# SunBangjie/FYP-BidirectionalPathTracer

Measured on AMD Instinct MI355X. Metric: Mrays/s + RMSE vs the scalar oracle, BDPT pass, Sponza-class scene 1920x1080 depth 8, higher is better.
Workload: dtype f32

## Files before the change

### fyp-bidirectionalpathtracer_amd/csrc/api.cpp

```cpp
#include <hip/hip_runtime.h>

#include <cmath>
#include <cstdio>
#include <cstdlib>
#include <cstring>
#include <future>
#include <functional>
#include <atomic>
#include <chrono>
#include <string>
#include <thread>
#include <vector>

#include "../../include/bdpt.h"
#include <new>

#include "bvh.h"
#include "kernels.h"
#include "refit.h"
#include "skin.h"
#include "scene_bvh.h"

using namespace bdpt;

namespace {
constexpr int kMaxStages = 64;
constexpr size_t kCountBlocks = 1;
constexpr size_t kHeadBlocks = 2;
constexpr size_t kLazyBlocks = kMaxLazyRounds + 2;
constexpr size_t kEyeCountBlock = kLazyBlocks - 1;
static_assert(kEyeCountBlock > (size_t)kMaxLazyRounds, "the eye list's cursor block must be one no lazy round uses");
constexpr size_t kCursorWords = (kCountBlocks + kHeadBlocks + kLazyBlocks) * kCursorBlock + 4 * kRayCursorBlock;
}

struct bdpt_ctx {
  int device = 0;
  int numCUs = 256;
  std::string err;
  bool haveScene = false, haveCamera = false, haveSize = false;
  SceneDev S{};
  std::vector<void*> sceneAllocs;
  bdpt_bvh_info bvhInfo{};
  bdpt_camera cam{};
  bdpt_environment env{};
  uint32_t W = 0, H = 0, maxDepth = 0;
  std::vector<std::pair<uint32_t, uint32_t>> rowRanges;
  uint32_t tileRows = 0;
  SplatLayout sl{1, 1, 0};
  bdpt_stripes stripes{0, 1, 0};
  PathBuf P{};
  std::vector<void*> frameAllocs;
  unsigned long long* splat = nullptr;
  unsigned long long* ownSplat = nullptr;
  DevCounters* counters = nullptr;
  hipStream_t lastStream = nullptr;
  bool timing = false;
  hipEvent_t ev[kMaxStages + 1]{};
  const char* stageNames[kMaxStages]{};
  int numStages = 0;
  bool evCreated = false;
  static constexpr int kMaxSideStages = 4;
  hipEvent_t sideEv[2 * kMaxSideStages]{};
  const char* sideNames[kMaxSideStages]{};
  int numSideStages = 0;
  int lazyRounds = 3;
  LaunchGrids grids{};
  int* stackOvf = nullptr;
  uint32_t stackOvfStride = 0;
  unsigned long long* rayCursor = nullptr;
  unsigned long long* adaptiveSum = nullptr;
  bdpt_gbuffer ownGb{};
  float4* bmfrPos[2] = {nullptr, nullptr};
  float4* bmfrNorm[2] = {nullptr, nullptr};
  float4* bmfrNoisy[2] = {nullptr, nullptr};
  float4* bmfrFiltered[2] = {nullptr, nullptr};
  uint8_t* bmfrAccept = nullptr;
  uint32_t* bmfrPrevPixel = nullptr;
  int bmfrRead = 0;
  hipStream_t walkStream = nullptr;
  hipEvent_t evFork = nullptr, evJoin = nullptr, evSplat = nullptr;
  uint32_t* hintPix = nullptr;
  bool hints = true;
  bdpt_camera hintCam{};
  bool hintCamValid = false;
  uint32_t numVertices = 0, numTriangles = 0;
  uint32_t* lightMaps = nullptr;
  bool refitReady = false;
  BvhRefitPlan refitPlan;
  RefitDev refit{};
  uint32_t numUpdates = 0;
  float* stage[3] = {nullptr, nullptr, nullptr};
  void* pinned = nullptr;
  size_t pinnedBytes = 0;
  hipEvent_t evStage = nullptr, evOrder = nullptr;
  bool stageInFlight = false;
  unsigned long long* groupSplat = nullptr;
  uint32_t groupSplatPlanes = 0;
  uint8_t* groupLightIdx = nullptr;
  const uint32_t* alphaTris = nullptr;
  uint32_t numAlphaTris = 0;
  bool areaReady = false;
  AreaDev area{};
  uint32_t areaTextured = 0;
  float* areaBlockSum = nullptr;
  uint32_t* areaBlockLast = nullptr;
  std::vector<void*> skinAllocs;
  bool haveSkin = false;
  SkinDev skin{};
  float* skinPalette[2] = {nullptr, nullptr};
};

namespace {

template <class F>
void hostParallelFor(size_t n, const F& f) {
  const int threads = bvhBuildThreads();
  if (threads <= 1 || n < 65536) {
    f((size_t)0, n);
    return;
  }
  WorkerScope pool;
  const size_t chunk = (n + (size_t)threads - 1) / (size_t)threads;
  for (int t = 1; t < threads; t++) {
    const size_t a = std::min(n, chunk * (size_t)t), b = std::min(n, a + chunk);
    if (a < b) pool.spawn([&f, a, b] { f(a, b); });
  }
  f((size_t)0, std::min(n, chunk));
  pool.join();
}

std::vector<uint32_t> alphaQuadPlane(const bdpt_texture& t) {
  std::vector<uint32_t> q((size_t)t.width * t.height);
  hostParallelFor(t.height, [&](size_t y0, size_t y1) { alphaQuadRows(t.rgba8, t.width, t.height, (uint32_t)y0, (uint32_t)y1, q.data()); });
  return q;
}

bool fail(bdpt_ctx* c, const std::string& m) {
  if (c) c->err = m;
  return false;
}
#define HIPCHK(ctx, expr)                                                                       \
  do {                                                                                          \
    hipError_t e_ = (expr);                                                                     \
    if (e_ != hipSuccess) {                                                                     \
      fail(ctx, std::string(#expr) + ": " + hipGetErrorString(e_));                             \
      return BDPT_E_HIP;                                                                        \
    }                                                                                           \
  } while (0)

template <class T>
int devAlloc(bdpt_ctx* c, std::vector<void*>& pool, T** out, size_t count) {
  void* p = nullptr;
  size_t bytes = std::max<size_t>(count * sizeof(T), 16);
  hipError_t e = hipMalloc(&p, bytes);
  if (e != hipSuccess) {
    fail(c, std::string("hipMalloc(") + std::to_string(bytes) + "): " + hipGetErrorString(e));
    return BDPT_E_NOMEM;
  }
  pool.push_back(p);
  *out = reinterpret_cast<T*>(p);
  return BDPT_OK;
}
template <class T>
int devUpload(bdpt_ctx* c, std::vector<void*>& pool, const T** out, const T* host, size_t count) {
  T* d = nullptr;
  int rc = devAlloc(c, pool, &d, count);
  if (rc) return rc;
  if (count) {
    std::string e;
    if (!bvhUploadStaged(d, host, count * sizeof(T), e)) {
      fail(c, e);
      return BDPT_E_HIP;
    }
  }
  *out = d;
  return BDPT_OK;
}
void freePool(std::vector<void*>& pool) {
  for (void* p : pool) (void)hipFree(p);
  pool.clear();
}
void freeLightGroups(bdpt_ctx* c) {
  if (c->groupSplat) (void)hipFree(c->groupSplat);
  if (c->groupLightIdx) (void)hipFree(c->groupLightIdx);
  c->groupSplat = nullptr;
  c->groupSplatPlanes = 0;
  c->groupLightIdx = nullptr;
}

#define ENTER(ctx) HIPCHK(ctx, hipSetDevice((ctx)->device))

bool streamIsCapturing(hipStream_t st) {
  hipStreamCaptureStatus cs = hipStreamCaptureStatusNone;
  if (hipStreamIsCapturing(st, &cs) != hipSuccess) return false;
  return cs != hipStreamCaptureStatusNone;
}

int allocOwnGbuffer(bdpt_ctx* c) {
  if (c->ownGb.worldPosition) return BDPT_OK;
  const size_t n = (size_t)c->W * c->H;
  const size_t mark = c->frameAllocs.size();
  bdpt_gbuffer g{};
  int rc;
  if ((rc = devAlloc(c, c->frameAllocs, &g.worldPosition, n * 4)) || (rc = devAlloc(c, c->frameAllocs, &g.worldNormal, n * 4)) ||
      (rc = devAlloc(c, c->frameAllocs, &g.materialDiffuse, n * 4)) || (rc = devAlloc(c, c->frameAllocs, &g.materialSpecRough, n * 4)) ||
      (rc = devAlloc(c, c->frameAllocs, &g.materialExtraParams, n * 4)) || (rc = devAlloc(c, c->frameAllocs, &g.emissive, n * 4))) {
    while (c->frameAllocs.size() > mark) {
      (void)hipFree(c->frameAllocs.back());
      c->frameAllocs.pop_back();
    }
    return rc;
  }
  c->ownGb = g;
  return BDPT_OK;
}

int allocBmfrHistory(bdpt_ctx* c) {
  if (c->bmfrAccept) return BDPT_OK;
  const size_t n = (size_t)c->W * c->H;
  const size_t mark = c->frameAllocs.size();
  float4 *pos[2]{}, *norm[2]{}, *noisy[2]{}, *filt[2]{};
  uint8_t* accept = nullptr;
  uint32_t* prevPixel = nullptr;
  int rc = BDPT_OK;
  for (int k = 0; k < 2 && !rc; k++) {
    if ((rc = devAlloc(c, c->frameAllocs, &pos[k], n)) || (rc = devAlloc(c, c->frameAllocs, &norm[k], n)) ||
        (rc = devAlloc(c, c->frameAllocs, &noisy[k], n)) || (rc = devAlloc(c, c->frameAllocs, &filt[k], n)))
      break;
  }
  if (!rc) rc = devAlloc(c, c->frameAllocs, &accept, n);
  if (!rc) rc = devAlloc(c, c->frameAllocs, &prevPixel, n);
  if (rc) {
    while (c->frameAllocs.size() > mark) {
      (void)hipFree(c->frameAllocs.back());
      c->frameAllocs.pop_back();
    }
    return rc;
  }
  for (int k = 0; k < 2; k++) {
    c->bmfrPos[k] = pos[k];
    c->bmfrNorm[k] = norm[k];
    c->bmfrNoisy[k] = noisy[k];
    c->bmfrFiltered[k] = filt[k];
  }
  c->bmfrAccept = accept;
  c->bmfrPrevPixel = prevPixel;
  return bdpt_bmfr_reset(c);
}

void stageMark(bdpt_ctx* c, hipStream_t st, const char* name) {
  if (!c->timing || c->numStages >= kMaxStages) return;
  c->stageNames[c->numStages] = name;
  c->numStages++;
  (void)hipEventRecord(c->ev[c->numStages], st);
}
void sideBegin(bdpt_ctx* c, hipStream_t side, const char* name) {
  if (!c->timing || c->numSideStages >= bdpt_ctx::kMaxSideStages) return;
  c->sideNames[c->numSideStages] = name;
  (void)hipEventRecord(c->sideEv[2 * c->numSideStages], side);
}
void sideEnd(bdpt_ctx* c, hipStream_t side) {
  if (!c->timing || c->numSideStages >= bdpt_ctx::kMaxSideStages) return;
  (void)hipEventRecord(c->sideEv[2 * c->numSideStages + 1], side);
  c->numSideStages++;
}

}

extern "C" {

int bdpt_create(int device_ordinal, bdpt_ctx** out_ctx) {
  if (!out_ctx) return BDPT_E_INVALID;
  *out_ctx = nullptr;
  int n = 0;
  if (hipGetDeviceCount(&n) != hipSuccess || n <= 0 || device_ordinal < 0 || device_ordinal >= n) return BDPT_E_HIP;
  if (hipSetDevice(device_ordinal) != hipSuccess) return BDPT_E_HIP;
  bdpt_ctx* c = new bdpt_ctx();
  c->device = device_ordinal;
  hipDeviceProp_t prop;
  if (hipGetDeviceProperties(&prop, device_ordinal) == hipSuccess && prop.multiProcessorCount > 0)
    c->numCUs = prop.multiProcessorCount;
  if (hipStreamCreateWithFlags(&c->walkStream, hipStreamNonBlocking) != hipSuccess ||
      hipEventCreateWithFlags(&c->evFork, hipEventDisableTiming) != hipSuccess ||
      hipEventCreateWithFlags(&c->evJoin, hipEventDisableTiming) != hipSuccess ||
      hipEventCreateWithFlags(&c->evSplat, hipEventDisableTiming) != hipSuccess ||
      hipEventCreateWithFlags(&c->evStage, hipEventDisableTiming) != hipSuccess ||
      hipEventCreateWithFlags(&c->evOrder, hipEventDisableTiming) != hipSuccess) {
    bdpt_destroy(c);
    return BDPT_E_HIP;
  }
  c->stackOvfStride = (uint32_t)c->numCUs * kMaxPersistentPerCU * kWave;
  if (kStackOvfRows > 0 &&
      hipMalloc(reinterpret_cast<void**>(&c->stackOvf), (size_t)kStackOvfRows * c->stackOvfStride * sizeof(int)) != hipSuccess) {
    bdpt_destroy(c);
    return BDPT_E_NOMEM;
  }
  if (hipMalloc(reinterpret_cast<void**>(&c->rayCursor), 2 * sizeof(unsigned long long)) != hipSuccess ||
      hipMemset(c->rayCursor, 0, 2 * sizeof(unsigned long long)) != hipSuccess ||
      hipMalloc(reinterpret_cast<void**>(&c->adaptiveSum), 2 * sizeof(unsigned long long)) != hipSuccess ||
      hipMemset(c->adaptiveSum, 0, 2 * sizeof(unsigned long long)) != hipSuccess) {
    bdpt_destroy(c);
    return BDPT_E_NOMEM;
  }
  bvhPrewarmStaging(device_ordinal);
  *out_ctx = c;
  return BDPT_OK;
}

void bdpt_destroy(bdpt_ctx* c) {
  if (!c) return;
  (void)hipSetDevice(c->device);
  (void)hipDeviceSynchronize();
  if (c->stackOvf) (void)hipFree(c->stackOvf);
  if (c->rayCursor) (void)hipFree(c->rayCursor);
  if (c->adaptiveSum) (void)hipFree(c->adaptiveSum);
  freeLightGroups(c);
  freePool(c->sceneAllocs);
  freePool(c->skinAllocs);
  freePool(c->frameAllocs);
  if (c->evCreated)
    for (int i = 0; i <= kMaxStages; i++) (void)hipEventDestroy(c->ev[i]);
  if (c->evCreated)
    for (hipEvent_t e : c->sideEv) (void)hipEventDestroy(e);
  if (c->evFork) (void)hipEventDestroy(c->evFork);
  if (c->evJoin) (void)hipEventDestroy(c->evJoin);
  if (c->evSplat) (void)hipEventDestroy(c->evSplat);
  if (c->evStage) (void)hipEventDestroy(c->evStage);
  if (c->evOrder) (void)hipEventDestroy(c->evOrder);
  if (c->pinned) (void)hipHostFree(c->pinned);
  if (c->walkStream) (void)hipStreamDestroy(c->walkStream);
  delete c;
}

const char* bdpt_last_error(const bdpt_ctx* c) { return c ? c->err.c_str() : "null context"; }

// ... 895 lines not shown
  c->lastStream = st;
  return BDPT_OK;
}

static_assert(sizeof(bdpt_light_sample) == 48 && sizeof(bdpt_light_emit) == 48 && offsetof(bdpt_light_sample, status) == 46,
              "the light query kernels write a record as three float4, light and status sharing the last word");
int bdpt_light_query(bdpt_ctx* c, const bdpt_light_desc* d, void* stream) {
  if (!c || !d) return BDPT_E_INVALID;
  if (!c->haveScene) {
    fail(c, "light_query: no scene (bdpt_set_scene first)");
    return BDPT_E_STATE;
  }
  const bool emitMode = d->mode == BDPT_LIGHT_EMIT;
  if (d->mode > BDPT_LIGHT_EMIT || d->matIndex > 1 || (d->flags & ~(BDPT_PARAM_AREA_LIGHTS | BDPT_LIGHT_USE_HINTS))) {
    fail(c, "light_query: unknown mode or flags, or matIndex > 1");
    return BDPT_E_INVALID;
  }
  const bool compact = d->compactRays || d->compactItems || d->compactCount;
  if (emitMode && (compact || (d->flags & BDPT_LIGHT_USE_HINTS))) {
    fail(c, "light_query: compaction and BDPT_LIGHT_USE_HINTS go with BDPT_LIGHT_NEE");
    return BDPT_E_INVALID;
  }
  if (compact && !(d->compactRays && d->compactItems && d->compactCount)) {
    fail(c, "light_query: compactRays, compactItems and compactCount go together");
    return BDPT_E_INVALID;
  }
  if (!d->num) return BDPT_OK;
  if (!aligned(d->seeds, 4) || (d->seedsOut && !aligned(d->seedsOut, 4)) || (d->numDevice && !aligned(d->numDevice, 4)) ||
      (emitMode ? !aligned(d->emits, 16) : (!aligned(d->surfaces, 16) || !aligned(d->samples, 16))) ||
      (compact && (!aligned(d->compactRays, 16) || !aligned(d->compactItems, 4) || !aligned(d->compactCount, 4)))) {
    fail(c, "light_query: surfaces, seeds, samples, emits or a compaction buffer missing or not aligned (records 16 bytes, words 4)");
    return BDPT_E_INVALID;
  }
  ENTER(c);
  hipStream_t st = reinterpret_cast<hipStream_t>(stream);
  AreaDev A{};
  if (d->flags & BDPT_PARAM_AREA_LIGHTS) {
    if (int rc = ensureAreaLights(c, st)) return rc;
    A = c->area;
  }
  if (int rc = orderAfterLast(c, st)) return rc;
  LightQueryDev Q{};
  Q.surf = reinterpret_cast<const float4*>(d->surfaces);
  Q.seeds = d->seeds;
  Q.seedsOut = d->seedsOut;
  Q.out = emitMode ? reinterpret_cast<float4*>(d->emits) : reinterpret_cast<float4*>(d->samples);
  Q.cap = d->num;
  Q.count = d->numDevice;
  Q.minT = d->minT;
  Q.compactRays = reinterpret_cast<float4*>(d->compactRays);
  Q.compactItems = d->compactItems;
  Q.compactCount = d->compactCount;
  launchLightQuery(c->S, Q, A, emitMode, d->matIndex == 0, (d->flags & BDPT_LIGHT_USE_HINTS) != 0, st);
  HIPCHK(c, hipGetLastError());
  c->lastStream = st;
  return BDPT_OK;
}

static_assert(sizeof(bdpt_connect_sample) == 48 && sizeof(bdpt_camera_sample) == 64 && offsetof(bdpt_connect_sample, status) == 44 &&
                  offsetof(bdpt_camera_sample, G) == 44 && offsetof(bdpt_camera_sample, pixel) == 48,
              "the connection query kernels write a record as three / four float4");
int bdpt_connect_query(bdpt_ctx* c, const bdpt_connect_desc* d, void* stream) {
  if (!c || !d) return BDPT_E_INVALID;
  if (!c->haveScene) {
    fail(c, "connect_query: no scene (bdpt_set_scene first)");
    return BDPT_E_STATE;
  }
  if (d->mode > BDPT_CONNECT_CAMERA || d->matIndex > 1 || d->flags || d->reserved) {
    fail(c, "connect_query: unknown mode, non-zero flags or reserved, or matIndex > 1");
    return BDPT_E_INVALID;
  }
  const bool camMode = d->mode == BDPT_CONNECT_CAMERA;
  if (camMode && !c->haveCamera) {
    fail(c, "connect_query: BDPT_CONNECT_CAMERA without a camera (bdpt_set_camera first)");
    return BDPT_E_STATE;
  }
  if (camMode && (!d->width || !d->height || (uint64_t)d->width * d->height >= (1ull << 32))) {
    fail(c, "connect_query: width and height must be > 0 with width * height < 2^32");
    return BDPT_E_INVALID;
  }
  const bool compact = d->compactRays || d->compactItems || d->compactCount;
  if (compact && !(d->compactRays && d->compactItems && d->compactCount)) {
    fail(c, "connect_query: compactRays, compactItems and compactCount go together");
    return BDPT_E_INVALID;
  }
  if (!d->num) return BDPT_OK;
  if (!aligned(d->light, 16) || (d->numDevice && !aligned(d->numDevice, 4)) ||
      (camMode ? !aligned(d->cameraSamples, 16)
               : (!aligned(d->eye, 16) || !aligned(d->samples, 16) || (d->eyePrev && !aligned(d->eyePrev, 16)) ||
                  (d->lightPrev && !aligned(d->lightPrev, 16)))) ||
      (compact && (!aligned(d->compactRays, 16) || !aligned(d->compactItems, 4) || !aligned(d->compactCount, 4)))) {
    fail(c, "connect_query: eye, light, samples, a predecessor or a compaction buffer missing or not aligned (records 16 bytes, words 4)");
    return BDPT_E_INVALID;
  }
  ENTER(c);
  hipStream_t st = reinterpret_cast<hipStream_t>(stream);
  if (int rc = orderAfterLast(c, st)) return rc;
  ConnectQueryDev Q{};
  Q.light = reinterpret_cast<const float4*>(d->light);
  Q.lightSpecular = d->lightSpecular;
  if (camMode) {
    Q.out = reinterpret_cast<float4*>(d->cameraSamples);
    Q.width = d->width;
    Q.height = d->height;
    Q.jitter[0] = d->pixelJitter[0];
    Q.jitter[1] = d->pixelJitter[1];
  } else {
    Q.eye = reinterpret_cast<const float4*>(d->eye);
    Q.eyePrev = reinterpret_cast<const float4*>(d->eyePrev);
    Q.lightPrev = reinterpret_cast<const float4*>(d->lightPrev);
    Q.eyeSpecular = d->eyeSpecular;
    Q.out = reinterpret_cast<float4*>(d->samples);
  }
  Q.cap = d->num;
  Q.count = d->numDevice;
  Q.minT = d->minT;
  Q.compactRays = reinterpret_cast<float4*>(d->compactRays);
  Q.compactItems = d->compactItems;
  Q.compactCount = d->compactCount;
  launchConnectQuery(Q, camMode ? &c->cam : nullptr, d->matIndex == 0, st);
  HIPCHK(c, hipGetLastError());
  c->lastStream = st;
  return BDPT_OK;
}

int bdpt_splat_add(bdpt_ctx* c, const bdpt_splat_desc* d, void* stream) {
  if (!c || !d) return BDPT_E_INVALID;
  if (!d->num) return BDPT_OK;
  if (!aligned(d->pixels, 4) || !aligned(d->values, 16) || !aligned(d->splat, 16) || (d->items && !aligned(d->items, 4)) ||
      (d->numDevice && !aligned(d->numDevice, 4))) {
    fail(c, "splat_add: pixels, values, splat, items or numDevice missing or not aligned (splat and values 16 bytes, words 4)");
    return BDPT_E_INVALID;
  }
  ENTER(c);
  hipStream_t st = reinterpret_cast<hipStream_t>(stream);
  if (int rc = orderAfterLast(c, st)) return rc;
  SplatAddDev A{};
  A.pixels = d->pixels;
  A.values = reinterpret_cast<const float4*>(d->values);
  A.visible = d->visible;
  A.items = d->items;
  A.splat = reinterpret_cast<unsigned long long*>(d->splat);
  A.numPixels = d->numPixels;
  A.cap = d->num;
  A.count = d->numDevice;
  launchSplatAdd(A, st);
  HIPCHK(c, hipGetLastError());
  c->lastStream = st;
  return BDPT_OK;
}

int bdpt_get_refit_info(bdpt_ctx* c, bdpt_refit_info* out) {
  if (!c || !out) return BDPT_E_INVALID;
  if (!c->haveScene) return BDPT_E_STATE;
  ENTER(c);
  *out = bdpt_refit_info{};
  out->sahCostBuilt = c->bvhInfo.sahCost;
  out->sahCost = c->bvhInfo.sahCost;
  out->numUpdates = c->numUpdates;
  if (c->numUpdates == 0) return BDPT_OK;
  HIPCHK(c, hipDeviceSynchronize());
  std::vector<float> area((size_t)c->refit.numNodes * 4);
  float root[6] = {0, 0, 0, 0, 0, 0};
  if (c->refit.numNodes) {
    HIPCHK(c, hipMemcpy(area.data(), c->refit.childArea, area.size() * sizeof(float), hipMemcpyDeviceToHost));
    HIPCHK(c, hipMemcpy(root, c->refit.box, sizeof(root), hipMemcpyDeviceToHost));
  }
  out->sahCost = bvhRefitSah(c->refitPlan, root, area.data());
  return BDPT_OK;
}

int bdpt_ctx_recs_hash(bdpt_ctx* c, uint64_t* out_hash) {
  if (!c || !out_hash) return BDPT_E_INVALID;
  if (!c->haveScene) return BDPT_E_STATE;
  ENTER(c);
  HIPCHK(c, hipDeviceSynchronize());
  std::vector<BvhRec> recs(c->S.numRecs);
  HIPCHK(c, hipMemcpy(recs.data(), c->S.recs, recs.size() * sizeof(BvhRec), hipMemcpyDeviceToHost));
  uint64_t h = 1469598103934665603ull;
  const uint8_t* b = reinterpret_cast<const uint8_t*>(recs.data());
  for (size_t i = 0; i < recs.size() * sizeof(BvhRec); i++) h = (h ^ b[i]) * 1099511628211ull;
  *out_hash = h;
  return BDPT_OK;
}

namespace {
int resizeRows(bdpt_ctx* c, uint32_t width, uint32_t height, uint32_t maxDepth);
}

int bdpt_resize(bdpt_ctx* c, uint32_t width, uint32_t height, bdpt_tile tile, uint32_t maxDepth) {
  if (!c) return BDPT_E_INVALID;
  if (!width || !height || tile.y0 > tile.y1 || tile.y1 > height) {
    fail(c, "resize: bad frame or tile");
    return BDPT_E_INVALID;
  }
  c->rowRanges.clear();
  if (tile.y1 > tile.y0) c->rowRanges.push_back({tile.y0, tile.y1});
  c->tileRows = tile.y1 - tile.y0;
  c->stripes = bdpt_stripes{0, 1, 0};
  c->sl = SplatLayout{1, 1, height};
  return resizeRows(c, width, height, maxDepth);
}

int bdpt_resize_stripes(bdpt_ctx* c, uint32_t width, uint32_t height, bdpt_stripes st, uint32_t maxDepth) {
  if (!c) return BDPT_E_INVALID;
  if (!width || !height || !st.stripeRows || !st.numOwners || st.owner >= st.numOwners) {
    fail(c, "resize_stripes: bad frame or stripe description");
    return BDPT_E_INVALID;
  }
  c->rowRanges.clear();
  c->tileRows = 0;
  const uint32_t numStripes = (height + st.stripeRows - 1) / st.stripeRows;
  for (uint32_t s = st.owner; s < numStripes; s += st.numOwners) {
    const uint32_t a = s * st.stripeRows, b = std::min(height, a + st.stripeRows);
    c->rowRanges.push_back({a, b});
    c->tileRows += b - a;
  }
  c->stripes = st;
  c->sl = SplatLayout{st.stripeRows, st.numOwners, ((numStripes + st.numOwners - 1) / st.numOwners) * st.stripeRows};
  return resizeRows(c, width, height, maxDepth);
}

uint32_t bdpt_stripe_rows(uint32_t height, uint32_t numOwners) {
  const uint32_t per = height / std::max(1u, numOwners * 4u);
  return std::max(1u, std::min(8u, per));
}
int bdpt_get_tile_info(const bdpt_ctx* c, bdpt_tile_info* out) {
  if (!c || !out) return BDPT_E_INVALID;
  if (!c->haveSize) return BDPT_E_STATE;
  out->numRows = c->tileRows;
  out->numPixels = c->P.Np;
  out->chunkRows = c->sl.chunkRows;
  out->numRowRanges = (uint32_t)c->rowRanges.size();
  out->splatU64 = (uint64_t)c->sl.owners * c->sl.chunkRows * c->W * 4;
  out->chunkU64 = (uint64_t)c->sl.chunkRows * c->W * 4;
  return BDPT_OK;
}

int bdpt_tile_row_ranges(const bdpt_ctx* c, uint32_t* out_first_last, uint32_t cap) {
  if (!c || !out_first_last) return BDPT_E_INVALID;
  if (!c->haveSize) return BDPT_E_STATE;
  const uint32_t n = std::min<uint32_t>(cap, (uint32_t)c->rowRanges.size());
  for (uint32_t i = 0; i < n; i++) {
    out_first_last[2 * i] = c->rowRanges[i].first;
    out_first_last[2 * i + 1] = c->rowRanges[i].second;
  }
  return (int)n;
}

namespace {
int resizeRows(bdpt_ctx* c, uint32_t width, uint32_t height, uint32_t maxDepth) {
  if (maxDepth > BDPT_MAX_DEPTH) {
    fail(c, "resize: maxDepth exceeds BDPT_MAX_DEPTH");
    return BDPT_E_LIMIT;
  }
  if ((uint64_t)width * height >= (1ull << 32) || (uint64_t)c->sl.owners * c->sl.chunkRows * width >= (1ull << 32)) {
    fail(c, "resize: frame too large");
    return BDPT_E_LIMIT;
  }
  if ((uint64_t)c->tileRows * width >= (1ull << 24)) {
    fail(c, "resize: a tile holds at most 2^24 - 1 pixels (path ids pack the pixel in 24 bits); render in smaller tiles");
    return BDPT_E_LIMIT;
  }
  HIPCHK(c, hipSetDevice(c->device));
  HIPCHK(c, hipDeviceSynchronize());
  freePool(c->frameAllocs);
  freeLightGroups(c);
  for (int k = 0; k < 2; k++) c->bmfrPos[k] = c->bmfrNorm[k] = c->bmfrNoisy[k] = c->bmfrFiltered[k] = nullptr;
  c->ownGb = bdpt_gbuffer{};
  c->bmfrAccept = nullptr;
  c->bmfrPrevPixel = nullptr;
  c->haveSize = false;
  c->W = width;
  c->H = height;
  c->maxDepth = maxDepth;
  PathBuf P{};
  P.Np = c->tileRows * width;
  P.D1 = std::max<uint32_t>(maxDepth, 1) + 1;
  const size_t np = std::max<uint32_t>(P.Np, 1);
  int rc;
  {
    std::vector<uint32_t> pix;
    pix.reserve(np);
    for (const auto& rr : c->rowRanges)
      for (uint32_t y = rr.first; y < rr.second; y++)
        for (uint32_t x = 0; x < width; x++) pix.push_back(y * width + x);
    if ((rc = devUpload(c, c->frameAllocs, &P.pix, pix.data(), pix.size()))) return rc;
  }
  if ((rc = devAlloc(c, c->frameAllocs, &P.v, (size_t)2 * P.D1 * NF4 * 4 * np))) return rc;
  if ((rc = devAlloc(c, c->frameAllocs, &P.rayDir, (size_t)6 * np))) return rc;
  if ((rc = devAlloc(c, c->frameAllocs, &P.seedE, np))) return rc;
  if ((rc = devAlloc(c, c->frameAllocs, &P.seedL, np))) return rc;
  if ((rc = devAlloc(c, c->frameAllocs, &P.eyeLast, np))) return rc;
  if ((rc = devAlloc(c, c->frameAllocs, &P.lightLast, np))) return rc;
  if ((rc = devAlloc(c, c->frameAllocs, &P.lightReal, np))) return rc;
  P.pathSubCap = (uint32_t)((((np + kWave - 1) / kWave + kNumSubQueues - 1) / kNumSubQueues + 1) * kWave);
  const size_t qcap = (size_t)P.pathSubCap * kNumSubQueues;
  for (int q = 0; q < 3; q++)
    if ((rc = devAlloc(c, c->frameAllocs, &P.queue[q], qcap))) return rc;
  if ((rc = devAlloc(c, c->frameAllocs, &P.qcount, (size_t)kCursorWords))) return rc;
  P.qhead = P.qcount + kCountBlocks * kCursorBlock;
  P.lazyCount = P.qhead + kHeadBlocks * kCursorBlock;
  P.rayCount = P.lazyCount + kLazyBlocks * kCursorBlock;
  P.rayHead = P.rayCount + 2 * kRayCursorBlock;
  {
    const uint32_t D = std::max<uint32_t>(maxDepth, 1);
    const uint64_t slots = (uint64_t)2 * D + numConnectPairs(D);
    const uint64_t blocks = (np + kWave - 1) / kWave;
    const uint64_t queueGridBlocks = (uint64_t)(P.pathSubCap / kWave) * kNumSubQueues;
    const uint64_t pairs = std::max<uint32_t>(numConnectPairs(D), 1);
    uint64_t subCapTerms = 0, subCapPairs = ((queueGridBlocks + kNumRaySubQueues - 1) / kNumRaySubQueues) * kWave * pairs;
    {
      const uint64_t G = D > 8 ? 16 : 8;
      const uint64_t perSub = (queueGridBlocks * G + kNumRaySubQueues - 1) / kNumRaySubQueues;
      subCapTerms = std::max<uint64_t>(subCapTerms, perSub * kWave * 2);
      subCapPairs = std::max<uint64_t>(subCapPairs, perSub * (kWave / G) * pairs);
    }
    (void)blocks;
    const uint64_t cap = (subCapTerms + subCapPairs) * kNumRaySubQueues;
    if (cap >= (1ull << 32) - 1) {
      fail(c, "resize: shadow-ray queue would exceed 2^32 entries; render in smaller tiles");
      return BDPT_E_LIMIT;
    }
    P.raySubCap[RAY_TERMS] = (uint32_t)subCapTerms;
    P.raySubCap[RAY_PAIRS] = (uint32_t)subCapPairs;
    P.rayBase[RAY_TERMS] = 0;
    P.rayBase[RAY_PAIRS] = (uint32_t)(subCapTerms * kNumRaySubQueues);
    P.rayCap = (uint32_t)cap;
    if ((rc = devAlloc(c, c->frameAllocs, &P.rayQ, (size_t)7 * cap))) return rc;
    if ((rc = devAlloc(c, c->frameAllocs, &P.rayContrib, (size_t)3 * cap))) return rc;
    if ((rc = devAlloc(c, c->frameAllocs, &P.rayVis, (size_t)cap))) return rc;
    if ((rc = devAlloc(c, c->frameAllocs, &P.slotRay, (size_t)slots * np))) return rc;
    if ((rc = devAlloc(c, c->frameAllocs, &P.splatPix, (size_t)D * np))) return rc;
    c->lazyRounds = np >= (1u << 18) ? 3 : 2;
    if (const char* e = std::getenv("BDPT_LAZY_ROUNDS")) {
      const int v = std::atoi(e);
      if (v >= 1 && v <= kMaxLazyRounds) c->lazyRounds = v;
    }
    const uint32_t batch = numConnectPairs(D);
    if ((rc = devAlloc(c, c->frameAllocs, &P.misE, (size_t)(D + 1) * np))) return rc;
    if ((rc = devAlloc(c, c->frameAllocs, &P.misL, (size_t)(D + 1) * np))) return rc;
    if ((rc = devAlloc(c, c->frameAllocs, &P.lazyCursor, np))) return rc;
    if ((rc = devAlloc(c, c->frameAllocs, &P.lazyRay, (size_t)std::max<uint32_t>(batch, 1) * np))) return rc;
  }
  c->hintPix = nullptr;
  c->hintCamValid = false;
  if (std::getenv("BDPT_NO_HINTS") == nullptr) {
    if ((rc = devAlloc(c, c->frameAllocs, &c->hintPix, (size_t)width * height))) return rc;
    HIPCHK(c, hipMemset(c->hintPix, 0xFF, (size_t)width * height * sizeof(uint32_t)));
  }
  const size_t splatU64 = (size_t)c->sl.owners * c->sl.chunkRows * width * 4;
  if ((rc = devAlloc(c, c->frameAllocs, &c->ownSplat, splatU64))) return rc;
  c->splat = c->ownSplat;
  if ((rc = devAlloc(c, c->frameAllocs, &c->counters, 1))) return rc;
  HIPCHK(c, hipMemset(c->splat, 0, splatU64 * sizeof(unsigned long long)));
  HIPCHK(c, hipMemset(c->counters, 0, sizeof(DevCounters)));
  c->P = P;
  if (!c->evCreated) {
    for (int i = 0; i <= kMaxStages; i++) HIPCHK(c, hipEventCreate(&c->ev[i]));
    for (hipEvent_t& e : c->sideEv) HIPCHK(c, hipEventCreate(&e));
    c->evCreated = true;
  }
  c->haveSize = true;
  return BDPT_OK;
}
}

int bdpt_gbuffer_execute(bdpt_ctx* c, const bdpt_gbuffer_params* gp, const bdpt_gbuffer* out, void* stream) {
  if (!c || !gp || !out) return BDPT_E_INVALID;
  if (!c->haveScene || !c->haveCamera || !c->haveSize) {
    fail(c, "gbuffer_execute: scene, camera and size must be set first");
    return BDPT_E_STATE;
  }
  if (!out->worldPosition || !out->worldNormal || !out->materialDiffuse || !out->materialSpecRough ||
      !out->materialExtraParams || !out->emissive) {
    fail(c, "gbuffer_execute: all six channels are required");
    return BDPT_E_INVALID;
  }
  ENTER(c);
  hipStream_t st = reinterpret_cast<hipStream_t>(stream);
  GBufferDev G{};
  G.cam = c->cam;
  G.gp = *gp;
  G.W = c->W;
  G.H = c->H;
  G.Np = c->P.Np;
  G.pix = c->P.pix;
  G.gb = *out;
  G.counters = nullptr;
  G.hintPix = c->hintPix;
  if (c->hintPix && c->tileRows != c->H && (!c->hintCamValid || std::memcmp(&c->hintCam, &c->cam, sizeof(bdpt_camera)) != 0)) {
    GBufferDev A = G;
    A.Np = c->W * c->H;
    A.pix = nullptr;
    launchHintFill(c->S, A, st);
    c->hintCam = c->cam;
    c->hintCamValid = true;
  }
  launchGBuffer(c->S, G, st);
  HIPCHK(c, hipGetLastError());
  c->lastStream = st;
  return BDPT_OK;
}

namespace {
int frameSetup(bdpt_ctx* c, const bdpt_params* p, const bdpt_gbuffer* in, float* out, hipStream_t st, FrameDev& F) {
  if (!c || !p || !out) return BDPT_E_INVALID;
  ENTER(c);
  if (!in) {
    if (!c->haveSize) {
      fail(c, "execute: scene, camera and size must be set first");
      return BDPT_E_STATE;
    }
    if (!c->ownGb.worldPosition) {
      if (streamIsCapturing(st)) {
        fail(c, "execute: the built-in primary stage needs bdpt_prepare(BDPT_PREPARE_PRIMARY) before stream capture");
        return BDPT_E_STATE;
      }
      if (int rc = allocOwnGbuffer(c)) return rc;
    }
    in = &c->ownGb;
  }
  if (!c->haveScene || !c->haveCamera || !c->haveSize) {
    fail(c, "execute: scene, camera and size must be set first");
    return BDPT_E_STATE;
  }
  if (p->maxDepth > c->maxDepth) {
    fail(c, "execute: params.maxDepth exceeds the depth given to bdpt_resize");
    return BDPT_E_LIMIT;
  }
  if (p->matIndex > 1) {
    fail(c, "execute: matIndex must be 0 (GGX) or 1 (Lambertian)");
    return BDPT_E_INVALID;
  }
  if (!in->worldPosition || !in->worldNormal || !in->materialDiffuse || !in->materialSpecRough || !in->emissive) {
    fail(c, "execute: G-buffer channels missing");
    return BDPT_E_INVALID;
  }
  F = FrameDev{};
  F.cam = c->cam;
  F.p = *p;
  F.W = c->W;
  F.H = c->H;
  F.sl = c->sl;
  F.out = out;
  F.splat = c->splat;
  F.gb = *in;
  F.counters = c->counters;
  F.envMap = c->env.envMap;
  F.envW = c->env.width;
  F.envH = c->env.height;
  for (int k = 0; k < 3; k++) F.envColor[k] = c->env.color[k];
  F.hintPix = c->hintPix;
  return BDPT_OK;
}

int connectionTail(bdpt_ctx* c, const FrameDev& F, hipStream_t st, const FrameVariant& V) {
  const PathBuf& P = c->P;
  const bdpt_params* p = &F.p;
  const int D = (int)p->maxDepth;
  if (!(p->flags & BDPT_PARAM_NO_CONNECT) && D >= 2) {
    const int nPairs = (int)numConnectPairs((uint32_t)D);
    const int b0 = (nPairs + kLazyBatchDiv - 1) / kLazyBatchDiv;
    int left = nPairs;
    for (int r = 0; r < c->lazyRounds && left > 0; r++) {
      const int batch = (r + 1 == c->lazyRounds) ? left : (b0 < left ? b0 : left);
      left -= batch;
      uint32_t* list = P.queue[1 + (r & 1)];
      uint32_t* next = P.queue[1 + ((r + 1) & 1)];
      HIPCHK(c, hipMemsetAsync(P.rayCount + (size_t)RAY_PAIRS * kRayCursorBlock, 0, kRayCursorBlock * sizeof(uint32_t), st));
      HIPCHK(c, hipMemsetAsync(P.rayHead + (size_t)RAY_PAIRS * kRayCursorBlock, 0, kRayCursorBlock * sizeof(uint32_t), st));
      launchLazyGen(F, P, list, P.lazyCount + (size_t)r * kCursorBlock, batch, st);
      stageMark(c, st, "lazy_gen");
      launchTraceShadow(c->S, F, P, RAY_PAIRS, c->grids, c->numCUs, st);
      stageMark(c, st, "lazy_trace");
      launchLazyCheck(F, P, V, list, P.lazyCount + (size_t)r * kCursorBlock, batch, next, P.lazyCount + (size_t)(r + 1) * kCursorBlock,
                      st);
    }
    stageMark(c, st, "lazy_check");
  }
  if (!(p->flags & BDPT_PARAM_DEFER_RESOLVE)) {
    launchFrameResolve(F, P, V, st);
    stageMark(c, st, V.kind == FrameKind::Groups ? "resolve_groups" : V.kind == FrameKind::Masked ? "resolve_masked" : "resolve");
  }
  HIPCHK(c, hipGetLastError());
  c->lastStream = st;
  return BDPT_OK;
}
}

namespace {
int executeFrame(bdpt_ctx* c, const bdpt_params* p, const bdpt_gbuffer* in, float* out, void* stream, const FrameVariant& V0,
                 bool groupsTakeArea = false) {
  FrameDev F;
  hipStream_t st = reinterpret_cast<hipStream_t>(stream);
  if (int rc = frameSetup(c, p, in, out, st, F)) return rc;
  FrameVariant V = V0;
  if (p->flags & BDPT_PARAM_AREA_LIGHTS) {
    if (p->flags & (BDPT_PARAM_MIS_POWER | BDPT_PARAM_MIS_LINEAR)) {
      fail(c, "execute: BDPT_PARAM_AREA_LIGHTS is not supported with BDPT_PARAM_MIS_POWER / _LINEAR");
      return BDPT_E_INVALID;
    }
    if (V.kind == FrameKind::Groups && !groupsTakeArea) {
      fail(c, "light groups: BDPT_PARAM_AREA_LIGHTS is not supported (the group planes have no slot for area lights)");
      return BDPT_E_INVALID;
    }
    if (int rc = ensureAreaLights(c, st)) return rc;
    V.area = c->area;
    if (V.kind == FrameKind::Groups && V.area.n) V.groups.areaW = V.area.total;
  }
  const PathBuf& P = c->P;
  PathBuf PE = P;
  if (V.kind == FrameKind::Masked) {
    PE.queue[0] = V.mask.eye;
    PE.qcount = V.mask.eyeCount;
  }
  if (!in) {
    bdpt_gbuffer_params gp{};
    gp.pixelJitter[0] = p->pixelJitter[0];
    gp.pixelJitter[1] = p->pixelJitter[1];
    gp.focalLen = 1.0f;
    gp.frameCount = p->frameCount;
    gp.envColor[0] = gp.envColor[1] = 0.5f;
    gp.envColor[2] = 0.8f;
    gp.envColor[3] = 1.0f;
    if (int rc = bdpt_gbuffer_execute(c, &gp, &c->ownGb, stream)) return rc;
  }

  c->numStages = 0;
  c->numSideStages = 0;
  if (c->timing) HIPCHK(c, hipEventRecord(c->ev[0], st));
  HIPCHK(c, hipMemsetAsync(P.qcount, 0, (size_t)kCursorWords * sizeof(uint32_t), st));
  HIPCHK(c, hipMemsetAsync(c->splat, 0, (size_t)c->sl.owners * c->sl.chunkRows * c->W * 4 * sizeof(unsigned long long), st));
  if (V.kind == FrameKind::Groups)
    HIPCHK(c, hipMemsetAsync(V.groups.splat, 0, (size_t)V.groups.numGroups * V.groups.framePix * 4 * sizeof(unsigned long long), st));
  if (!(p->flags & BDPT_PARAM_KEEP_COUNTERS)) HIPCHK(c, hipMemsetAsync(c->counters, 0, sizeof(DevCounters), st));
  stageMark(c, st, "clear");

  launchInitPaths(c->S, F, P, V, st);
  stageMark(c, st, "init_paths");

  launchWalk(c->S, F, P, V, c->grids, c->numCUs, st);
  stageMark(c, st, "walk");

  const bool mis = (p->flags & (BDPT_PARAM_MIS_POWER | BDPT_PARAM_MIS_LINEAR)) != 0;
  if (mis) {
    launchMisPrefix(F, P, st);
    stageMark(c, st, "mis_prefix");
    launchGenNee(c->S, F, PE, V.area, st);
    stageMark(c, st, "gen_nee");
    launchGenSplat(c->S, F, P, st);
    stageMark(c, st, "gen_splat");
    launchGenConnect(c->S, F, PE, st);
    stageMark(c, st, "gen_connect");
    launchTraceShadow(c->S, F, P, RAY_TERMS, c->grids, c->numCUs, st);
    stageMark(c, st, "trace_terms");
  } else {
    HIPCHK(c, hipEventRecord(c->evFork, st));
    HIPCHK(c, hipStreamWaitEvent(c->walkStream, c->evFork, 0));
    sideBegin(c, c->walkStream, "side:gen_splat");
    launchGenSplat(c->S, F, P, c->walkStream);
    sideEnd(c, c->walkStream);
    HIPCHK(c, hipEventRecord(c->evSplat, c->walkStream));
    sideBegin(c, c->walkStream, "side:gen_connect");
    launchGenConnect(c->S, F, PE, c->walkStream);
    sideEnd(c, c->walkStream);
    HIPCHK(c, hipEventRecord(c->evJoin, c->walkStream));
    launchGenNee(c->S, F, PE, V.area, st);
    stageMark(c, st, "gen_nee");
    HIPCHK(c, hipStreamWaitEvent(st, c->evSplat, 0));
    stageMark(c, st, "splat_wait");
    launchTraceShadow(c->S, F, P, RAY_TERMS, c->grids, c->numCUs, st);
    stageMark(c, st, "trace_terms");
    HIPCHK(c, hipStreamWaitEvent(st, c->evJoin, 0));
    stageMark(c, st, "connect_wait");
  }
  launchTraceShadow(c->S, F, P, RAY_PAIRS, c->grids, c->numCUs, st);
  stageMark(c, st, "trace_pairs");
  launchGather(F, P, V, P.queue[1], P.lazyCount, st);
  stageMark(c, st, "gather");
  if (p->flags & BDPT_PARAM_DEFER_TAIL) {
    HIPCHK(c, hipGetLastError());
    c->lastStream = st;
    return BDPT_OK;
  }
  return connectionTail(c, F, st, V);
}

int allocLightGroups(bdpt_ctx* c, hipStream_t st, uint32_t planes) {
  if (c->groupSplat && c->groupSplatPlanes >= planes) return BDPT_OK;
  if (streamIsCapturing(st)) {
    fail(c, "light groups: the splat planes need bdpt_prepare(BDPT_PREPARE_LIGHT_GROUPS / _LIGHT_GROUP_TABLE) before stream capture");
    return BDPT_E_STATE;
  }
  if (c->groupSplat) {
    HIPCHK(c, hipDeviceSynchronize());
    freeLightGroups(c);
  }
  const size_t n = (size_t)c->W * c->H;
  void *sp = nullptr, *li = nullptr;
  if (hipMalloc(&sp, std::max<size_t>((size_t)planes * n * 4 * sizeof(unsigned long long), 16)) != hipSuccess ||
      hipMalloc(&li, std::max<size_t>(c->P.Np, 16)) != hipSuccess) {
    if (sp) (void)hipFree(sp);
    fail(c, "light groups: hipMalloc of the splat planes failed");
    return BDPT_E_NOMEM;
  }
  c->groupSplat = reinterpret_cast<unsigned long long*>(sp);
  c->groupSplatPlanes = planes;
  c->groupLightIdx = reinterpret_cast<uint8_t*>(li);
  return BDPT_OK;
}

int wholeFrameCheck(bdpt_ctx* c, const bdpt_params* p, const std::string& what) {
  if (p && (p->flags & (BDPT_PARAM_DEFER_RESOLVE | BDPT_PARAM_DEFER_TAIL))) {
    fail(c, what + ": BDPT_PARAM_DEFER_RESOLVE and BDPT_PARAM_DEFER_TAIL are not supported");
    return BDPT_E_INVALID;
  }
  if (!c->haveScene || !c->haveSize) {
    fail(c, what + ": scene and size must be set first");
    return BDPT_E_STATE;
  }
  if (c->stripes.stripeRows != 0 || c->tileRows != c->H) {
    fail(c, what + ": the context must render the whole frame (no tile, no stripes)");
    return BDPT_E_INVALID;
  }
  return BDPT_OK;
}
}

int bdpt_execute(bdpt_ctx* c, const bdpt_params* p, const bdpt_gbuffer* in, float* out, void* stream) {
  return executeFrame(c, p, in, out, stream, FrameVariant{});
}

int bdpt_execute_light_groups(bdpt_ctx* c, const bdpt_params* p, const bdpt_gbuffer* in, float* out, float* groups, void* stream) {
  if (!c) return BDPT_E_INVALID;
  if (!groups) {
    fail(c, "light groups: groups is NULL");
    return BDPT_E_INVALID;
  }
  if (int rc = wholeFrameCheck(c, p, "light groups")) return rc;
  ENTER(c);
  hipStream_t st = reinterpret_cast<hipStream_t>(stream);
  if (int rc = allocLightGroups(c, st, c->S.numLights)) return rc;
  FrameVariant V;
  V.kind = FrameKind::Groups;
  V.groups.planes = groups;
  V.groups.splat = c->groupSplat;
  V.groups.lightIdx = c->groupLightIdx;
  V.groups.numLights = c->S.numLights;
  V.groups.numGroups = c->S.numLights;
  V.groups.framePix = (uint64_t)c->W * c->H;
  for (uint32_t i = 0; i < c->S.numLights; i++) V.groups.groupOf[i] = (uint8_t)i;
  return executeFrame(c, p, in, out, stream, V);
}

int bdpt_execute_grouped(bdpt_ctx* c, const bdpt_params* p, const bdpt_gbuffer* in, float* out, const bdpt_light_group_desc* d,
                         void* stream) {
  if (!c) return BDPT_E_INVALID;
  if (!p || !out) {
    fail(c, "execute_grouped: params or out is NULL");
    return BDPT_E_INVALID;
  }
  if (!d || !d->planes || !d->groupOf) {
    fail(c, "execute_grouped: the descriptor, its planes or its groupOf is NULL");
    return BDPT_E_INVALID;
  }
  if (int rc = wholeFrameCheck(c, p, "execute_grouped")) return rc;
  if (d->numGroups < 1 || d->numGroups > BDPT_MAX_LIGHTS + 1) {
    fail(c, "execute_grouped: numGroups must be 1 .. BDPT_MAX_LIGHTS + 1");
    return BDPT_E_INVALID;
  }
  const bool area = (p->flags & BDPT_PARAM_AREA_LIGHTS) != 0;
  const uint32_t numLights = c->S.numLights;
  if (d->numAssigned != numLights + (area ? 1u : 0u)) {
    fail(c, "execute_grouped: numAssigned must be numLights, or numLights + 1 with BDPT_PARAM_AREA_LIGHTS");
    return BDPT_E_INVALID;
  }
  for (uint32_t i = 0; i < d->numAssigned; i++)
    if (d->groupOf[i] >= d->numGroups) {
      fail(c, "execute_grouped: groupOf[" + std::to_string(i) + "] is not below numGroups");
      return BDPT_E_INVALID;
    }
  if (d->reserved[0] || d->reserved[1]) {
    fail(c, "execute_grouped: reserved must be 0");
    return BDPT_E_INVALID;
  }
  if (area && (p->flags & (BDPT_PARAM_MIS_POWER | BDPT_PARAM_MIS_LINEAR))) {
    fail(c, "execute: BDPT_PARAM_AREA_LIGHTS is not supported with BDPT_PARAM_MIS_POWER / _LINEAR");
    return BDPT_E_INVALID;
  }
  ENTER(c);
  hipStream_t st = reinterpret_cast<hipStream_t>(stream);
  if (int rc = allocLightGroups(c, st, d->numGroups)) return rc;
  FrameVariant V;
  V.kind = FrameKind::Groups;
  V.groups.planes = d->planes;
  V.groups.splat = c->groupSplat;
  V.groups.lightIdx = c->groupLightIdx;
  V.groups.numLights = numLights;
  V.groups.numGroups = d->numGroups;
  V.groups.framePix = (uint64_t)c->W * c->H;
  for (uint32_t i = 0; i < d->numAssigned; i++) V.groups.groupOf[i] = d->groupOf[i];
  return executeFrame(c, p, in, out, stream, V, true);
}

int bdpt_execute_masked(bdpt_ctx* c, const bdpt_params* p, const bdpt_gbuffer* in, const uint8_t* mask, float* out, void* stream) {
  if (!c) return BDPT_E_INVALID;
  if (!mask) {
    fail(c, "execute_masked: mask is NULL");
    return BDPT_E_INVALID;
  }
  if (int rc = wholeFrameCheck(c, p, "execute_masked")) return rc;
  const PathBuf& P = c->P;
  const bool misOn = p && (p->flags & (BDPT_PARAM_MIS_POWER | BDPT_PARAM_MIS_LINEAR)) != 0;
  FrameVariant V;
  V.kind = FrameKind::Masked;
  V.mask.mask = mask;
  V.mask.eye = P.queue[2];
  V.mask.eyeCount = P.lazyCount + kEyeCountBlock * kCursorBlock;
  V.mask.walkEye = misOn ? P.queue[0] : V.mask.eye;
  V.mask.walkEyeCount = misOn ? P.qcount : V.mask.eyeCount;
  return executeFrame(c, p, in, out, stream, V);
}

namespace {
int adaptiveSetup(bdpt_ctx* c, const bdpt_adaptive_state* s, const char* what, AdaptiveDev& A) {
  if (!s || !s->mean || !s->m2 || !s->count || !s->mask || !s->active) {
    fail(c, std::string(what) + ": a state buffer is NULL");
    return BDPT_E_INVALID;
  }
  if (int rc = wholeFrameCheck(c, nullptr, what)) return rc;
  if (reinterpret_cast<uintptr_t>(s->mean) % 16 != 0) {
    fail(c, std::string(what) + ": mean must be 16-byte aligned (RGBA32F)");
    return BDPT_E_INVALID;
  }
  A = AdaptiveDev{};
  A.mean = reinterpret_cast<float4*>(s->mean);
  A.m2 = s->m2;
  A.count = s->count;
  A.mask = s->mask;
  A.active = s->active;
  A.W = c->W;
  A.H = c->H;
  return BDPT_OK;
}
}

int bdpt_adaptive_reset(bdpt_ctx* c, const bdpt_adaptive_state* s, void* stream) {
  if (!c) return BDPT_E_INVALID;
  AdaptiveDev A;
  if (int rc = adaptiveSetup(c, s, "adaptive_reset", A)) return rc;
  ENTER(c);
  launchAdaptiveReset(A, reinterpret_cast<hipStream_t>(stream));
  HIPCHK(c, hipGetLastError());
  return BDPT_OK;
}

int bdpt_adaptive_update(bdpt_ctx* c, const bdpt_adaptive_params* a, const bdpt_adaptive_state* s, float* frame, void* stream) {
  if (!c) return BDPT_E_INVALID;
  if (!a || !frame) {
    fail(c, "adaptive_update: params or frame is NULL");
    return BDPT_E_INVALID;
  }
  const uint32_t b = a->blockSize;
  if (b != 1 && b != 2 && b != 4 && b != 8 && b != 16) {
    fail(c, "adaptive_update: blockSize must be 1, 2, 4, 8 or 16");
    return BDPT_E_INVALID;
  }
  if (a->minSamples < 2 || a->maxSamples < a->minSamples) {
    fail(c, "adaptive_update: need 2 <= minSamples <= maxSamples");
    return BDPT_E_INVALID;
  }
  if (reinterpret_cast<uintptr_t>(frame) % 16 != 0) {
    fail(c, "adaptive_update: frame must be 16-byte aligned (RGBA32F)");
    return BDPT_E_INVALID;
  }
  AdaptiveDev A;
  if (int rc = adaptiveSetup(c, s, "adaptive_update", A)) return rc;
  A.frame = reinterpret_cast<float4*>(frame);
  A.threshold = a->threshold;
  A.epsilon = a->epsilon;
  A.minSamples = a->minSamples;
  A.maxSamples = a->maxSamples;
  A.blockSize = b;
  ENTER(c);
  hipStream_t st = reinterpret_cast<hipStream_t>(stream);
  if (int rc = orderAfterLast(c, st)) return rc;
  launchAdaptiveUpdate(A, c->adaptiveSum, st);
  HIPCHK(c, hipGetLastError());
  c->lastStream = st;
  return BDPT_OK;
}

int bdpt_execute_tail(bdpt_ctx* c, const bdpt_params* p, const bdpt_gbuffer* in, float* out, void* stream) {
  FrameDev F;
  hipStream_t st = reinterpret_cast<hipStream_t>(stream);
  if (int rc = frameSetup(c, p, in, out, st, F)) return rc;
  stageMark(c, st, "tail_wait");
  return connectionTail(c, F, st, FrameVariant{});
}

int bdpt_prepare(bdpt_ctx* c, uint32_t what) {
  if (!c) return BDPT_E_INVALID;
  if ((what & ~(BDPT_PREPARE_REFIT | BDPT_PREPARE_AREA_LIGHTS)) || !what) {
    if (!c->haveSize) {
      fail(c, "prepare: bdpt_resize must be called first");
      return BDPT_E_STATE;
    }
  }
  if ((what & BDPT_PREPARE_REFIT) && !c->haveScene) {
    fail(c, "prepare: BDPT_PREPARE_REFIT needs a scene");
    return BDPT_E_STATE;
  }
  if ((what & BDPT_PREPARE_AREA_LIGHTS) && !c->haveScene) {
    fail(c, "prepare: BDPT_PREPARE_AREA_LIGHTS needs a scene");
    return BDPT_E_STATE;
  }
  if ((what & (BDPT_PREPARE_LIGHT_GROUPS | BDPT_PREPARE_LIGHT_GROUP_TABLE)) && !c->haveScene) {
    fail(c, "prepare: BDPT_PREPARE_LIGHT_GROUPS needs a scene (the planes are per light)");
    return BDPT_E_STATE;
  }
  ENTER(c);
  if (what & BDPT_PREPARE_REFIT)
    if (int rc = ensureRefit(c, nullptr)) return rc;
  if (what & BDPT_PREPARE_PRIMARY)
    if (int rc = allocOwnGbuffer(c)) return rc;
  if (what & BDPT_PREPARE_BMFR)
    if (int rc = allocBmfrHistory(c)) return rc;
  if (what & (BDPT_PREPARE_LIGHT_GROUPS | BDPT_PREPARE_LIGHT_GROUP_TABLE))
    if (int rc = allocLightGroups(c, nullptr, c->S.numLights + ((what & BDPT_PREPARE_LIGHT_GROUP_TABLE) ? 1u : 0u))) return rc;
  if (what & BDPT_PREPARE_AREA_LIGHTS)
    if (int rc = ensureAreaLights(c, nullptr)) return rc;
  return BDPT_OK;
}

int bdpt_bmfr_execute(bdpt_ctx* c, const bdpt_bmfr_params* p, const bdpt_gbuffer* g, float* noisy, void* stream) {
  if (!c || !p || !g || !noisy) return BDPT_E_INVALID;
  if (!c->haveSize) {
    fail(c, "bmfr: bdpt_resize must be called first");
    return BDPT_E_STATE;
  }
  if (!g->worldPosition || !g->worldNormal || !g->materialDiffuse) {
    fail(c, "bmfr: WorldPosition, WorldNormal and MaterialDiffuse are required");
    return BDPT_E_INVALID;
  }
  ENTER(c);
  hipStream_t st = reinterpret_cast<hipStream_t>(stream);
  const size_t n = (size_t)c->W * c->H;
  if (!c->bmfrAccept) {
    if (streamIsCapturing(st)) {
      fail(c, "bmfr: the history needs bdpt_prepare(BDPT_PREPARE_BMFR) before stream capture");
      return BDPT_E_STATE;
    }
    if (int rc = allocBmfrHistory(c)) return rc;
  }
  BmfrDev A{};
  A.W = c->W;
  A.H = c->H;
  A.frame = p->frameNumber;
  A.full = (p->flags & BDPT_BMFR_FULL_FRAME) ? 1u : 0u;
  A.doPre = (p->flags & BDPT_BMFR_PREPROCESS) ? 1u : 0u;
  for (int k = 0; k < 16; k++) A.m[k] = p->prevViewProj[k];
  A.curPos = reinterpret_cast<const float4*>(g->worldPosition);
  A.curNorm = g->worldNormal;
  A.albedo = g->materialDiffuse;
  A.noisy = reinterpret_cast<float4*>(noisy);
  const int r = c->bmfrRead, w = 1 - r;
  A.prevPosR = c->bmfrPos[r];
  A.prevNormR = c->bmfrNorm[r];
  A.prevNoisyR = c->bmfrNoisy[r];
  A.prevFilteredR = c->bmfrFiltered[r];
  A.prevPosW = c->bmfrPos[w];
  A.prevNormW = c->bmfrNorm[w];
  A.prevNoisyW = c->bmfrNoisy[w];
  A.prevFilteredW = c->bmfrFiltered[w];
  A.accept = c->bmfrAccept;
  A.prevPixel = c->bmfrPrevPixel;
  if (!(p->flags & BDPT_BMFR_POSTPROCESS))
    HIPCHK(c, hipMemcpyAsync(c->bmfrFiltered[w], c->bmfrFiltered[r], n * sizeof(float4), hipMemcpyDeviceToDevice, st));
  launchBmfr(A, p->flags, st);
// ... 463 lines not shown
```

### fyp-bidirectionalpathtracer_amd/csrc/kernels.h

```cpp
#pragma once
#include <hip/hip_runtime.h>
#include <stdint.h>

#include "../../include/bdpt.h"
#include "texture_planes.h"

namespace bdpt {

constexpr int kWave = 64;
#ifndef KSTACK
#define KSTACK 32
#endif
constexpr int kStackEntries = KSTACK;
#ifndef BDPT_STACK_LDS
#define BDPT_STACK_LDS 24
#endif
constexpr int kStackLds = BDPT_STACK_LDS < KSTACK ? BDPT_STACK_LDS : KSTACK;
constexpr int kMaxPersistentPerCU = 32;
constexpr int kStackOvfRows = KSTACK - kStackLds;
constexpr int kShadeRecF4 = 7;
constexpr uint32_t kNoRay = 0xFFFFFFFFu;
constexpr uint32_t kNumSubQueues = 32;
#ifndef BDPT_FETCH_CHUNK
#define BDPT_FETCH_CHUNK 256
#endif
constexpr uint32_t kFetchChunk = BDPT_FETCH_CHUNK;
constexpr uint32_t kCursorStride = 32;
constexpr uint32_t kCursorBlock = kNumSubQueues * kCursorStride;
#ifndef BDPT_RAY_SUBQUEUES
#define BDPT_RAY_SUBQUEUES 32
#endif
constexpr uint32_t kNumRaySubQueues = BDPT_RAY_SUBQUEUES;
constexpr uint32_t kRayCursorBlock = kNumRaySubQueues * kCursorStride;
constexpr uint32_t kCounterShards = 64;

enum : int { F_COL = 0, F_POS = 3, F_N = 6, F_V = 9, F_DIF = 12, F_SPEC = 15, F_ROUGH = 18, F_ISSPEC = 19, F_PDF = 20, NF = 21 };
constexpr int NF4 = 6;
enum : int { PATH_EYE = 0, PATH_LIGHT = 1 };
enum : int { RAY_TERMS = 0, RAY_PAIRS = 1 };

struct TexDev {
  const uint8_t* px;
  uint32_t w, h, srgb, pow2;
};

struct SceneConst {
  bdpt_light lights[BDPT_MAX_LIGHTS];
  float srgbLut[256];
};

struct SceneDev {
  const uint4* recs;
  const float4* shade;
  const float* bitangents;
  const uint32_t* indices;
  const bdpt_material* materials;
  const TexDev* textures;
  const TexDev* matTex;
  const SceneConst* sc;
  uint32_t numLights;
  uint32_t hasBitangents;
  uint32_t numRecs;
  const float4* alphaRecs;
  int* stackOvf;
  uint32_t stackOvfStride;
  const uint32_t* lightMap;
  uint32_t lightMapRes;
};

struct DevCounters {
  unsigned long long v[kCounterShards][32];
};
enum : int {
  C_RAYS_PRIMARY = 0, C_RAYS_EYE, C_RAYS_LIGHT, C_RAYS_NEE, C_RAYS_SPLAT, C_RAYS_CONNECT,
  C_NODE_CLOSEST, C_TRI_CLOSEST, C_NODE_SHADOW, C_TRI_SHADOW, C_PIX_VALID, C_SPLATS, C_RAYS_LAZY,
  C_STACK_MAX,
  C_ALPHA_CLOSEST, C_ALPHA_SHADOW,
  C_HINT_NEE, C_HINT_SPLAT
};

inline __host__ __device__ uint32_t numConnectPairs(uint32_t D) {
  uint32_t n = 0;
  for (uint32_t t = 2; t <= D; t++) n += (t < D - 1) ? t : (D - 1);
  return n;
}

struct PathBuf {
  float* v;
  float* rayDir;
  const uint32_t* pix;
  uint32_t* seedE;
  uint32_t* seedL;
  uint8_t* eyeLast;
  uint8_t* lightLast;
  uint8_t* lightReal;
  uint32_t* queue[3];
  uint32_t pathSubCap;
  uint32_t* qcount;
  uint32_t* qhead;
  float* rayQ;
  float* rayContrib;
  uint8_t* rayVis;
  uint32_t* rayCount;
  uint32_t* rayHead;
  uint32_t raySubCap[2];
  uint32_t rayBase[2];
  uint32_t* slotRay;
  uint32_t* splatPix;
  float* misE;
  float* misL;
  uint8_t* lazyCursor;
  uint32_t* lazyRay;
  uint32_t* lazyCount;
  uint32_t rayCap;
  uint32_t Np, D1;
};

struct SplatLayout {
  uint32_t stripeRows, owners, chunkRows;
};
inline __host__ __device__ size_t splatIndex(const SplatLayout& L, uint32_t W, uint32_t x, uint32_t y) {
  const uint32_t s = y / L.stripeRows;
  const uint32_t owner = s % L.owners, row = (s / L.owners) * L.stripeRows + (y - s * L.stripeRows);
  return ((size_t)owner * L.chunkRows + row) * W + x;
}

struct FrameDev {
  bdpt_camera cam;
  bdpt_params p;
  uint32_t W, H;
  SplatLayout sl;
  float* out;
  unsigned long long* splat;
  bdpt_gbuffer gb;
  DevCounters* counters;
  const float* envMap;
  uint32_t envW, envH;
  float envColor[3];
  const uint32_t* hintPix;
};

struct GroupDev {
  float* planes;
  unsigned long long* splat;
  uint8_t* lightIdx;
  uint32_t numLights;
  uint32_t numGroups;
  uint64_t framePix;
  const float* areaW;
  uint8_t groupOf[BDPT_MAX_LIGHTS + 1];
};

struct MaskDev {
  const uint8_t* mask;
  uint32_t* eye;
  uint32_t* eyeCount;
  const uint32_t* walkEye;
  const uint32_t* walkEyeCount;
};

constexpr uint32_t kNoAlphaRec = 0xFFFFFFFFu;
struct BvhRefitNode;
struct AreaDev {
  const float* cdf;
  const float4* emit;
  const float* total;
  uint32_t n;
};

enum class FrameKind { Plain, Groups, Masked };
struct FrameVariant {
  FrameKind kind = FrameKind::Plain;
  GroupDev groups{};
  MaskDev mask{};
  AreaDev area{};
};

struct GBufferDev {
  bdpt_camera cam;
  bdpt_gbuffer_params gp;
  uint32_t W, H, Np;
  const uint32_t* pix;
  bdpt_gbuffer gb;
  DevCounters* counters;
  uint32_t* hintPix;
};

struct BmfrDev {
  uint32_t W, H, frame;
  uint32_t full, doPre;
  float m[16];
  const float4* curPos;
  const uint16_t* curNorm;
  const uint16_t* albedo;
  float4* noisy;
  const float4 *prevPosR, *prevNormR, *prevNoisyR, *prevFilteredR;
  float4 *prevPosW, *prevNormW, *prevNoisyW, *prevFilteredW;
  uint8_t* accept;
  uint32_t* prevPixel;
};
void launchBmfr(const BmfrDev& A, uint32_t flags, hipStream_t st);

void launchGBuffer(const SceneDev& S, const GBufferDev& G, hipStream_t st);
void launchAlphaRecs(const SceneDev& S, const uint32_t* alphaTris, uint32_t n, const unsigned long long* quadByTex, float4* out, hipStream_t st);
void launchHintFill(const SceneDev& S, const GBufferDev& G, hipStream_t st);
void launchLightMaps(const SceneDev& S, uint32_t* maps, uint32_t res, hipStream_t st);
void launchInitPaths(const SceneDev& S, const FrameDev& F, const PathBuf& P, const FrameVariant& V, hipStream_t st);
struct LaunchGrids {
  uint32_t walk[16] = {};
  uint32_t shadow[2] = {0, 0};
  uint32_t rays[3] = {0, 0, 0};
};
void launchWalk(const SceneDev& S, const FrameDev& F, const PathBuf& P, const FrameVariant& V, LaunchGrids& G, int numCUs,
                hipStream_t st);
void launchMisPrefix(const FrameDev& F, const PathBuf& P, hipStream_t st);
void launchGenNee(const SceneDev& S, const FrameDev& F, const PathBuf& P, const AreaDev& A, hipStream_t st);
void launchGenSplat(const SceneDev& S, const FrameDev& F, const PathBuf& P, hipStream_t st);
void launchGenConnect(const SceneDev& S, const FrameDev& F, const PathBuf& P, hipStream_t st);
void launchTraceShadow(const SceneDev& S, const FrameDev& F, const PathBuf& P, int rayClass, LaunchGrids& G, int numCUs, hipStream_t st);
void launchTraceRays(const SceneDev& S, const float4* rays, uint32_t cap, const uint32_t* count, unsigned long long* cursor, int mode,
                     float4* hits, uint8_t* vis, LaunchGrids& G, int numCUs, hipStream_t st);
void launchCameraRays(const bdpt_camera& cam, const bdpt_gbuffer_params& gp, uint32_t W, uint32_t H, float4* rays, hipStream_t st);
void launchShadeHits(const SceneDev& S, uint32_t numTris, const float4* rays, const float4* hits, uint32_t cap, const uint32_t* count,
                     bool normalMap, float4* out, hipStream_t st);
void launchBsdfQuery(const float4* surf, uint32_t cap, const uint32_t* count, bool eval, bool ggx, bool fromLobe, const uint32_t* seeds,
                     const float4* dirs, float4* out, hipStream_t st);
struct LightQueryDev {
  const float4* surf;
  const uint32_t* seeds;
  uint32_t* seedsOut;
  float4* out;
  uint32_t cap;
  const uint32_t* count;
  float minT;
  float4* compactRays;
  uint32_t* compactItems;
  uint32_t* compactCount;
};
void launchLightQuery(const SceneDev& S, const LightQueryDev& Q, const AreaDev& A, bool emitMode, bool ggx, bool hints, hipStream_t st);
struct ConnectQueryDev {
  const float4* eye;
  const float4* light;
  const float4* eyePrev;
  const float4* lightPrev;
  const uint8_t* eyeSpecular;
  const uint8_t* lightSpecular;
  float4* out;
  uint32_t cap;
  const uint32_t* count;
  float minT;
  uint32_t width, height;
  float jitter[2];
  float4* compactRays;
  uint32_t* compactItems;
  uint32_t* compactCount;
};
void launchConnectQuery(const ConnectQueryDev& Q, const bdpt_camera* cam, bool ggx, hipStream_t st);
struct SplatAddDev {
  const uint32_t* pixels;
  const float4* values;
  const uint8_t* visible;
  const uint32_t* items;
  unsigned long long* splat;
  uint32_t numPixels;
  uint32_t cap;
  const uint32_t* count;
};
void launchSplatAdd(const SplatAddDev& A, hipStream_t st);
void launchGather(const FrameDev& F, const PathBuf& P, const FrameVariant& V, uint32_t* lazyList, uint32_t* lazyCount, hipStream_t st);
void launchLazyGen(const FrameDev& F, const PathBuf& P, const uint32_t* list, const uint32_t* listCount, int batch, hipStream_t st);
void launchLazyCheck(const FrameDev& F, const PathBuf& P, const FrameVariant& V, const uint32_t* list, const uint32_t* listCount,
                     int batch, uint32_t* nextList, uint32_t* nextCount, hipStream_t st);
constexpr int kLazyBatchDiv = 8;
constexpr int kMaxLazyRounds = 8;
void launchResolve(const unsigned long long* splat, bool tileLocal, uint32_t splatRow0, const SplatLayout& L, float* out, uint32_t W,
                   const uint32_t* pix, uint32_t Np, hipStream_t st);
void launchFrameResolve(const FrameDev& F, const PathBuf& P, const FrameVariant& V, hipStream_t st);
struct AdaptiveDev {
  float4* mean;
  float* m2;
  uint32_t* count;
  uint8_t* mask;
  uint32_t* active;
  float4* frame;
  uint32_t W, H;
  float threshold, epsilon;
  uint32_t minSamples, maxSamples, blockSize;
};
void launchAdaptiveUpdate(const AdaptiveDev& A, unsigned long long* scratch, hipStream_t st);
void launchAdaptiveReset(const AdaptiveDev& A, hipStream_t st);
void launchAccumulate(float* last, float* cur, uint32_t accumCount, uint32_t maxAccum, uint64_t numTexels, hipStream_t st);
void launchAccumulateTile(float* last, float* cur, uint32_t accumCount, uint32_t maxAccum, const uint32_t* pix, uint32_t Np,
                          hipStream_t st);
void launchTilePack(const void* frame, void* packed, uint32_t bytesPerPixel, const uint32_t* pix, uint32_t Np, hipStream_t st);
void launchTileUnpack(const void* packed, void* frame, uint32_t bytesPerPixel, uint32_t W, uint32_t H, uint32_t stripeRows, uint32_t owners,
                      uint32_t owner, uint32_t packedRows, hipStream_t st);
void launchTestRng(const uint32_t* v0, const uint32_t* v1, uint32_t n, uint32_t draws, uint32_t* states, float* floats,
                   hipStream_t st);
void launchTestTrace(const SceneDev& S, const float* rays, uint32_t n, int mode, int32_t* prim, float* tuv, hipStream_t st);
void launchTestTraceShadow(const SceneDev& S, const float* planes, uint32_t cap, const uint32_t* count, uint32_t* head, uint8_t* vis,
                           DevCounters* counters, float tmin, int numCUs, hipStream_t st);
void launchTestBsdf(const float* in, uint32_t n, uint32_t matIndex, float* out, hipStream_t st);

void launchAreaMarkReferenced(const BvhRefitNode* nodes, uint32_t numNodes, const uint4* recs, uint8_t* referenced, hipStream_t st);
void launchAreaCount(const SceneDev& S, uint32_t numTris, const uint8_t* referenced, uint32_t* blockCount, uint32_t* blockBase,
                     uint32_t* counts, hipStream_t st);
void launchAreaCompact(const SceneDev& S, uint32_t numTris, const uint8_t* referenced, const uint32_t* blockBase,
                       const uint32_t* alphaTris, uint32_t numAlphaTris, float4* emit, hipStream_t st);
void launchAreaRefresh(const SceneDev& S, const AreaDev& A, float* blockSum, uint32_t* blockLast, hipStream_t st);
void launchTestAreaSample(const SceneDev& S, const AreaDev& A, int mode, const uint32_t* states, const float* points, uint32_t n,
                          float* out, hipStream_t st);

}
```

### fyp-bidirectionalpathtracer_amd/csrc/kernels.hip

```cpp
#include "kernels.h"

#include <algorithm>
#include <type_traits>

#include "device_area.hpp"
#include "device_connect.hpp"
#include "device_math.hpp"
#include "device_scene.hpp"
#include "device_trace.hpp"
#include "launch.hpp"

namespace bdpt {

#define BD __device__ __forceinline__

BD void wavePush(bool active, uint32_t value, uint32_t* items, uint32_t* count, uint32_t subCap, uint32_t q = 0xffffffffu) {
  unsigned long long mask = __ballot(active);
  if (mask == 0ull) return;
  const int lane = (int)(threadIdx.x & 63u);
  const int leader = __ffsll((long long)mask) - 1;
  if (q == 0xffffffffu) q = blockIdx.x % kNumSubQueues;
  uint32_t base = 0;
  if (lane == leader) base = atomicAdd(&count[q * kCursorStride], (uint32_t)__popcll(mask));
  base = (uint32_t)__shfl((int)base, leader);
  const uint32_t prefix = (uint32_t)__popcll(mask & ((1ull << lane) - 1ull));
  if (active) items[q * subCap + base + prefix] = value;
}
BD bool queueChunk(const uint32_t* count, uint32_t subCap, bool& act, uint32_t& idx) {
  const uint32_t q = blockIdx.x % kNumSubQueues, c0 = (blockIdx.x / kNumSubQueues) * kWave;
  const uint32_t n = count[q * kCursorStride];
  if (c0 >= n) return false;
  const uint32_t i = c0 + threadIdx.x;
  act = i < n;
  idx = q * subCap + i;
  return true;
}

constexpr int kVtxQ = NF4;
BD float4* vtxPtr(const PathBuf& P, int path, int k, uint32_t p) {
  return reinterpret_cast<float4*>(P.v) + ((size_t)(path * (int)P.D1 + k) * P.Np + p) * kVtxQ;
}
BD constexpr int fieldQ(int f) { return f == F_POS ? 0 : f == F_N ? 1 : f == F_DIF ? 2 : f == F_SPEC ? 3 : f == F_COL ? 4 : 5; }
BD f3 ldPlane3(const PathBuf& P, int path, int k, int f, uint32_t p) {
  const float4 q = vtxPtr(P, path, k, p)[fieldQ(f)];
  return f3{q.x, q.y, q.z};
}
BD float ldPlane1(const PathBuf& P, int path, int k, int f, uint32_t p) {
  const int q = (f == F_ROUGH) ? 0 : (f == F_ISSPEC ? 1 : 2);
  return reinterpret_cast<const float*>(vtxPtr(P, path, k, p))[q * 4 + 3];
}

struct Vtx {
  f3 color, pos, N, V, dif, spec;
  float rough;
  bool isSpec;
  float pdf;
};
BD Vtx zeroVtx() {
  Vtx v;
  v.color = v.pos = v.N = v.V = v.dif = v.spec = mk(0);
  v.rough = 0.0f;
  v.isSpec = false;
  v.pdf = 0.0f;
  return v;
}
BD void storeVtx(const PathBuf& P, int path, int k, uint32_t p, const Vtx& v) {
  float4* r = vtxPtr(P, path, k, p);
  const float4 q0 = make_float4(v.pos.x, v.pos.y, v.pos.z, v.rough), q1 = make_float4(v.N.x, v.N.y, v.N.z, v.isSpec ? 1.0f : 0.0f),
               q2 = make_float4(v.dif.x, v.dif.y, v.dif.z, v.pdf), q3 = make_float4(v.spec.x, v.spec.y, v.spec.z, 0.0f),
               q4 = make_float4(v.color.x, v.color.y, v.color.z, 0.0f), q5 = make_float4(v.V.x, v.V.y, v.V.z, 0.0f);
  r[0] = q0;
  r[1] = q1;
  r[2] = q2;
  r[3] = q3;
  r[4] = q4;
  r[5] = q5;
}
template <bool GGX = true>
BD void loadSurf(const PathBuf& P, int path, int k, uint32_t p, Vtx& v) {
  const float4* r = vtxPtr(P, path, k, p);
  const float4 q0 = r[0], q1 = r[1], q2 = r[2];
  v.pos = mk(q0.x, q0.y, q0.z);
  v.N = mk(q1.x, q1.y, q1.z);
  v.dif = mk(q2.x, q2.y, q2.z);
  v.pdf = q2.w;
  if (GGX) {
    const float4 q3 = r[3];
    v.spec = mk(q3.x, q3.y, q3.z);
    v.rough = q0.w;
    v.isSpec = q1.w != 0.0f;
  } else {
    v.spec = mk(0);
    v.rough = 0.0f;
    v.isSpec = false;
  }
}

BD void unpackHalf4(const uint16_t* base, size_t idx, float& a, float& b, float& c, float& d) {
  const uint2 raw = reinterpret_cast<const uint2*>(base)[idx];
  a = f16_to_f32((uint16_t)(raw.x & 0xffffu));
  b = f16_to_f32((uint16_t)(raw.x >> 16));
  c = f16_to_f32((uint16_t)(raw.y & 0xffffu));
  d = f16_to_f32((uint16_t)(raw.y >> 16));
}
BD void packHalf4(uint16_t* base, size_t idx, float a, float b, float c, float d) {
  uint2 raw;
  raw.x = (uint32_t)f32_to_f16(a) | ((uint32_t)f32_to_f16(b) << 16);
  raw.y = (uint32_t)f32_to_f16(c) | ((uint32_t)f32_to_f16(d) << 16);
  reinterpret_cast<uint2*>(base)[idx] = raw;
}

BD float atan2_WAR(float y, float x) {
  if (x > 0.f)
    return det_atan(y / x);
  else if (x < 0.f && y >= 0.f)
    return det_atan(y / x) + kPi;
  else if (x < 0.f && y < 0.f)
    return det_atan(y / x) - kPi;
  else if (x == 0.f && y > 0.f)
    return kPi / 2.f;
  else if (x == 0.f && y < 0.f)
    return -kPi / 2.f;
  return 0.f;
}

BD f3 envLookup(const float* envMap, uint32_t envW, uint32_t envH, f3 d) {
  const f3 pd = normalize(d);
  const float u = (1.f + atan2_WAR(pd.x, -pd.z) * kInvPi) * 0.5f;
  const float v = det_acos(pd.y) * kInvPi;
  const uint32_t ex = (uint32_t)(u * (float)envW), ey = (uint32_t)(v * (float)envH);
  f3 c = mk(0);
  if (ex < envW && ey < envH) c = ld3(envMap + ((size_t)ey * envW + ex) * 4);
  return c;
}

template <bool COUNT, bool HINT_ONLY = false>
__global__ __launch_bounds__(kWave) void gbuffer_kernel(SceneDev S, GBufferDev G) {
  BDPT_ONE_WAVE_PER_GROUP();
  __shared__ int s_stack[kStackEntries * kWave];
  const uint32_t p = blockIdx.x * kWave + threadIdx.x;
  if (p >= G.Np) return;
  const size_t pix = HINT_ONLY ? (size_t)p : (size_t)G.pix[p];
  const uint32_t y = (uint32_t)(pix / G.W), x = (uint32_t)(pix - (size_t)y * G.W);

  const f3 camPos = ld3(G.cam.posW);
  f3 o, d;
  primaryRay(G.cam, G.gp, x, y, G.W, G.H, o, d);

  uint32_t nNodes = 0, nTris = 0;
  Hit h = traverse<1, COUNT>(S, o, d, 0.0f, 1e+38f, s_stack + threadIdx.x, nNodes, nTris);
  if (COUNT) {
    addCount(G.counters, C_RAYS_PRIMARY, 1);
    addCount(G.counters, C_NODE_CLOSEST, nNodes);
    addCount(G.counters, C_TRI_CLOSEST, nTris);
  }
  float4* oP = reinterpret_cast<float4*>(G.gb.worldPosition);
  if (G.hintPix) G.hintPix[pix] = (h.prim < 0) ? kNoHint : h.rec;
  if (HINT_ONLY) return;
  if (h.prim < 0) {
    const f3 c = G.gp.envMap ? envLookup(G.gp.envMap, G.gp.envWidth, G.gp.envHeight, d) : ld3(G.gp.envColor);
    oP[pix] = make_float4(0, 0, 0, 0);
    packHalf4(G.gb.worldNormal, pix, 0, 0, 0, 0);
    packHalf4(G.gb.materialDiffuse, pix, c.x, c.y, c.z, 1.0f);
    packHalf4(G.gb.materialSpecRough, pix, 0, 0, 0, 0);
    packHalf4(G.gb.materialExtraParams, pix, 0, 0, 0, 0);
    packHalf4(G.gb.emissive, pix, 0, 0, 0, 0);
    return;
  }
  Shading sd = shadeHit<true>(S, (uint32_t)h.prim, h.u, h.v, camPos);
  oP[pix] = make_float4(sd.posW.x, sd.posW.y, sd.posW.z, 1.0f);
  packHalf4(G.gb.worldNormal, pix, sd.N.x, sd.N.y, sd.N.z, length(sd.posW - camPos));
  packHalf4(G.gb.materialDiffuse, pix, sd.diffuse.x, sd.diffuse.y, sd.diffuse.z, sd.opacity);
  packHalf4(G.gb.materialSpecRough, pix, sd.specular.x, sd.specular.y, sd.specular.z, sd.linearRoughness);
  packHalf4(G.gb.materialExtraParams, pix, sd.IoR, 0, 0, 0);
  packHalf4(G.gb.emissive, pix, sd.emissive.x, sd.emissive.y, sd.emissive.z, 0);
}

__global__ __launch_bounds__(kWave) void light_map_kernel(SceneDev S, uint32_t* __restrict__ maps, uint32_t res) {
  BDPT_ONE_WAVE_PER_GROUP();
  __shared__ int s_stack[kStackEntries * kWave];
  const uint32_t perLight = 6u * res * res;
  const uint32_t i = blockIdx.x * kWave + threadIdx.x;
  if (i >= perLight * S.numLights) return;
  const uint32_t light = i / perLight, t = i - light * perLight;
  const bdpt_light& l = S.sc->lights[light];
  uint32_t out = kNoHint;
  if (l.type != BDPT_LIGHT_DIRECTIONAL) {
    const uint32_t face = t / (res * res), iv = (t / res) % res, iu = t % res;
    const float uc = (((float)iu + 0.5f) / (float)res) * 2.0f - 1.0f, vc = (((float)iv + 0.5f) / (float)res) * 2.0f - 1.0f;
    const float m = (face & 1u) ? -1.0f : 1.0f;
    const f3 d = (face < 2u) ? mk(m, uc, vc) : ((face < 4u) ? mk(uc, m, vc) : mk(uc, vc, m));
    uint32_t nNodes = 0, nTris = 0;
    const Hit h = traverse<0, false>(S, ld3(l.posW), d, 0.0f, 1.0e38f, s_stack + threadIdx.x, nNodes, nTris);
    if (h.prim >= 0) out = h.rec;
  }
  maps[i] = out;
}

struct NoArg {};
template <FrameKind V>
using FrameArg = std::conditional_t<V == FrameKind::Groups, GroupDev, std::conditional_t<V == FrameKind::Masked, MaskDev, NoArg>>;
template <class A>
BD GroupDev groupOf(const A&) { return GroupDev{}; }
BD const GroupDev& groupOf(const GroupDev& g) { return g; }
template <class A>
BD MaskDev maskOf(const A&) { return MaskDev{}; }
BD const MaskDev& maskOf(const MaskDev& m) { return m; }

template <bool GGX, bool GROUPS, bool MASKED, bool AREA = false>
BD void initPathsLane(const SceneDev& S, const FrameDev& F, const PathBuf& P, const GroupDev& Gr, const MaskDev& M,
                      const AreaDev& A = AreaDev{}) {
  const uint32_t p = blockIdx.x * kWave + threadIdx.x;
  const bool inTile = p < P.Np;
  const size_t pix = inTile ? P.pix[p] : 0;
  bool geom = false;
  const bool active = !MASKED || (inTile && M.mask[pix] != 0);
  float4* out4 = reinterpret_cast<float4*>(F.out);
  if (inTile) {
    const float4 wp = reinterpret_cast<const float4*>(F.gb.worldPosition)[pix];
    float dr, dg, db, da;
    unpackHalf4(F.gb.materialDiffuse, pix, dr, dg, db, da);
    geom = (wp.w != 0.0f);
    if (!geom) {
      if (active) out4[pix] = make_float4(dr, dg, db, 1.0f);
      P.eyeLast[p] = 0;
      if (GROUPS) {
        float4* g4 = reinterpret_cast<float4*>(Gr.planes) + pix;
        for (uint32_t k = 0; k < Gr.numGroups; k++) g4[(size_t)k * Gr.framePix] = make_float4(0.0f, 0.0f, 0.0f, 1.0f);
        g4[(size_t)Gr.numGroups * Gr.framePix] = make_float4(dr, dg, db, 1.0f);
      }
    } else {
      float nx, ny, nz, nw, sr, sg, sb, sa, er, eg, eb, ea;
      unpackHalf4(F.gb.worldNormal, pix, nx, ny, nz, nw);
      unpackHalf4(F.gb.materialSpecRough, pix, sr, sg, sb, sa);
      unpackHalf4(F.gb.emissive, pix, er, eg, eb, ea);
      const f3 camPos = ld3(F.cam.posW);
      const f3 worldPos = mk(wp.x, wp.y, wp.z), worldNorm = mk(nx, ny, nz), dif = mk(dr, dg, db), spec = mk(sr, sg, sb);
      const float roughness = sa * sa;
      const f3 V = normalize(camPos - worldPos);
      uint32_t seed = initRand((uint32_t)pix, F.p.frameCount);
      P.seedE[p] = seed;
      f3 outDir;
      float pdf;
      bool isSpec;
      f3 thr = sampleBRDF<GGX>(seed, worldNorm, worldNorm, V, dif, spec, roughness,
                               (F.p.flags & BDPT_PARAM_SPECULAR_FROM_LOBE) != 0, outDir, pdf, isSpec);
      Vtx v;
      v.color = thr;
      v.pos = worldPos;
      v.N = worldNorm;
      v.V = V;
      v.dif = dif;
      v.spec = spec;
      v.rough = roughness;
      v.isSpec = isSpec;
      v.pdf = pdf;
      storeVtx(P, PATH_EYE, 1, p, v);
      float* rd = P.rayDir + (size_t)(PATH_EYE * 3) * P.Np + p;
      rd[0] = outDir.x;
      rd[P.Np] = outDir.y;
      rd[2 * (size_t)P.Np] = outDir.z;

      const float areaW = AREA ? areaTotal(A) : 0.0f;
      const int lightsCount = (int)S.numLights + ((AREA && areaW > 0.0f) ? 1 : 0);
      int index = (int)(nextRand(seed) * (float)lightsCount);
      if (index > lightsCount - 1) index = lightsCount - 1;
      if (GROUPS) Gr.lightIdx[p] = (uint8_t)index;
      f3 lightDir;
      Vtx lv = zeroVtx();
      if (AREA && index == (int)S.numLights) {
        f3 n;
        lv.pos = areaLightStart(S, A, areaW, seed, n, lightDir, lv.color).pos;
      } else {
        const bdpt_light& l = S.sc->lights[index];
        if (l.type == BDPT_LIGHT_DIRECTIONAL)
          lightDir = ld3(l.dirW);
        else
          lightDir = sampleUnitSphere(seed);
        lightDir = getCosHemisphereSample(seed, lightDir);
        lv.pos = ld3(l.posW);
        lv.color = ld3(l.intensity);
      }
      lv.pdf = 1.0f / (float)lightsCount;
      storeVtx(P, PATH_LIGHT, 0, p, lv);
      float* rl = P.rayDir + (size_t)(PATH_LIGHT * 3) * P.Np + p;
      rl[0] = lightDir.x;
      rl[P.Np] = lightDir.y;
      rl[2 * (size_t)P.Np] = lightDir.z;
      P.seedL[p] = seed;

      const uint8_t D = (uint8_t)F.p.maxDepth;
      P.eyeLast[p] = D < 1 ? 1 : D;
      P.lightLast[p] = D;
      P.lightReal[p] = D;
      const bool em = (er > 0.0f) || (eg > 0.0f) || (eb > 0.0f);
      if (active) out4[pix] = em ? make_float4(0.0f + er, 0.0f + eg, 0.0f + eb, 0.0f + ea) : make_float4(0, 0, 0, 0);
    }
  }
  wavePush(geom, p, P.queue[0], P.qcount, P.pathSubCap);
  if (MASKED) wavePush(geom && active, p, M.eye, M.eyeCount, P.pathSubCap);
}
template <bool GGX, FrameKind V>
__global__ __launch_bounds__(kWave) void init_paths_kernel(SceneDev S, FrameDev F, PathBuf P, FrameArg<V> A) {
  BDPT_ONE_WAVE_PER_GROUP();
  initPathsLane<GGX, V == FrameKind::Groups, V == FrameKind::Masked>(S, F, P, groupOf(A), maskOf(A));
}
template <bool GGX, FrameKind V>
__global__ __launch_bounds__(kWave) void init_paths_area_kernel(SceneDev S, FrameDev F, PathBuf P, FrameArg<V> A, AreaDev E) {
  BDPT_ONE_WAVE_PER_GROUP();
  initPathsLane<GGX, V == FrameKind::Groups, V == FrameKind::Masked, true>(S, F, P, groupOf(A), maskOf(A), E);
}

constexpr uint32_t kPoolEntries = 128;
#ifndef BDPT_WALK_ORDER
#define BDPT_WALK_ORDER 1
#endif
#ifndef BDPT_WALK_SHADE_MIN
#define BDPT_WALK_SHADE_MIN 64
#endif
#ifndef BDPT_WALK_LEAF_WAIT
#define BDPT_WALK_LEAF_WAIT 1
#endif
#ifndef BDPT_WALK_NODE_BURST
#define BDPT_WALK_NODE_BURST 3
#endif
#ifndef BDPT_WALK_CHUNK
#define BDPT_WALK_CHUNK 64
#endif
#ifndef BDPT_WALK_REFILL
#define BDPT_WALK_REFILL BDPT_REFILL_IDLE
#endif
BD uint32_t packPath(uint32_t p, int path, int k) { return p | ((uint32_t)path << 24) | ((uint32_t)k << 25); }

#ifndef BDPT_WALK_WAVES_PER_EU
#define BDPT_WALK_WAVES_PER_EU 4
#endif
#ifndef BDPT_WALK_STACK_LDS
#define BDPT_WALK_STACK_LDS kStackEntries
#endif
constexpr int kWalkStackLds = BDPT_WALK_STACK_LDS;
constexpr uint32_t kParkedMiss = 1u << 30;
template <bool GGX, bool COUNT, bool EXT, bool MASKED>
__global__ __launch_bounds__(kWave) __attribute__((amdgpu_waves_per_eu(BDPT_WALK_WAVES_PER_EU, 8))) void walk_kernel(
    SceneDev S, FrameDev F, PathBuf P, uint32_t* __restrict__ head, FrameArg<MASKED ? FrameKind::Masked : FrameKind::Plain> mask) {
  BDPT_ONE_WAVE_PER_GROUP();
  __shared__ int s_stack[kWalkStackLds * kWave];
  __shared__ uint4 s_pool[kPoolEntries];
  const MaskDev& M = maskOf(mask);
  int* stk = s_stack + threadIdx.x;
  const int lane = (int)(threadIdx.x & 63u);
  const unsigned long long laneBelow = (1ull << lane) - 1ull;
  const int D = (int)F.p.maxDepth;
  const bool fromLobe = (F.p.flags & BDPT_PARAM_SPECULAR_FROM_LOBE) != 0;
  const uint32_t firstV = (D >= 2) ? 0u : kNumSubQueues, numV = 2u * kNumSubQueues - firstV;
  bool trav = false;
  uint32_t id = 0;
  TravState T;
  travInit(T, mk(0), mk(0), F.p.minT, 1.0e38f);
  T.cur = kDone;
  uint32_t nNodes = 0, nTris = 0, nAlpha = 0;
  uint32_t nEye = 0, nLight = 0, nParked = 0, nReady = 0;
  uint32_t vq = firstV + blockIdx.x % numV, tried = 0, chunkPos = 0, chunkEnd = 0, chunk = BDPT_WALK_CHUNK;
  bool exhausted = false;
  const uint32_t wavesPerList = (gridDim.x + numV - 1) / numV;
  for (;;) {
    unsigned long long travMask = __ballot(trav);
    const bool flush = (travMask == 0ull) && nReady == 0 && exhausted && nParked > 0;
    if (nParked >= (uint32_t)BDPT_WALK_SHADE_MIN || flush) {
      const uint32_t n = nParked < (uint32_t)kWave ? nParked : (uint32_t)kWave;
      nParked -= n;
      const bool act = (uint32_t)lane < n;
      uint4 rec = make_uint4(0, 0, 0, 0);
      if (act) rec = s_pool[nParked + (uint32_t)lane];
      __syncthreads();
      const uint32_t p = rec.x & 0xffffffu;
      const int path = (int)((rec.x >> 24) & 1u), k = (int)((rec.x >> 25) & 31u);
      nEye += (uint32_t)__popcll(__ballot(act && path == PATH_EYE));
      nLight += (uint32_t)__popcll(__ballot(act && path == PATH_LIGHT));
      bool survive = false;
      f3 L = mk(0);
      if (act) {
        const bool miss = EXT ? (rec.x & kParkedMiss) != 0u : (int)rec.y < 0;
        const int prim = miss ? -1 : (int)rec.y;
        const f3 o = ldPlane3(P, path, k, F_POS, p);
        f3 found = mk(0);
        bool haveFound = false;
        if (prim >= 0) {
          const uint32_t seed = (path == PATH_EYE) ? P.seedE[p] : P.seedL[p];
          const f3 thr = ldPlane3(P, path, k, F_COL, p);
          Shading sd = shadeHit<false>(S, (uint32_t)prim, __uint_as_float(rec.z), __uint_as_float(rec.w), o);
          float pdf;
          bool isSpec;
          f3 w = sampleBRDF<GGX>(seed, sd.N, sd.N, sd.V, sd.diffuse, sd.specular, sd.roughness, fromLobe, L, pdf, isSpec);
          Vtx v;
          v.color = thr * w;
          v.pos = sd.posW;
          v.N = sd.N;
          v.V = sd.V;
          v.dif = sd.diffuse;
          v.spec = sd.specular;
          v.rough = sd.roughness;
          v.isSpec = isSpec;
          v.pdf = pdf;
          storeVtx(P, path, k + 1, p, v);
          survive = (k + 2 <= D);
          if (EXT && path == PATH_EYE && (F.p.flags & BDPT_PARAM_EMISSIVE_HITS) &&
              (sd.emissive.x > 0.0f || sd.emissive.y > 0.0f || sd.emissive.z > 0.0f)) {
            found = thr * sd.emissive;
            haveFound = true;
          }
        } else {
          if (EXT && path == PATH_EYE && (F.p.flags & BDPT_PARAM_ENV_ON_MISS)) {
            const f3 dir = mk(__uint_as_float(rec.y), __uint_as_float(rec.z), __uint_as_float(rec.w));
            const f3 env = F.envMap ? envLookup(F.envMap, F.envW, F.envH, dir) : ld3(F.envColor);
            found = ldPlane3(P, path, k, F_COL, p) * env;
            haveFound = true;
          }
          Vtx g = zeroVtx();
          if (path == PATH_EYE && k == 1) {
            g.pos = o;
          } else {
            loadSurf(P, path, k, p, g);
            g.V = ldPlane3(P, path, k, F_V, p);
            if (path == PATH_LIGHT && k == 0) g.pdf = 0.0f;
          }
          g.color = mk(0);
          storeVtx(P, path, k + 1, p, g);
          if (path == PATH_EYE) {
            P.eyeLast[p] = (uint8_t)(k + 1);
          } else {
            P.lightLast[p] = (uint8_t)(k + 1);
            P.lightReal[p] = (uint8_t)k;
          }
        }
        if (MASKED && haveFound && M.mask[P.pix[p]] == 0) haveFound = false;
        if (EXT && haveFound) {
          f3 term = clampVec(found / (float)(k + 1), F.p.clampUpper);
          if (isnan3(term)) term = mk(0);
          float4* out4 = reinterpret_cast<float4*>(F.out);
          const size_t pix = P.pix[p];
          float4 acc = out4[pix];
          acc.x = acc.x + term.x;
          acc.y = acc.y + term.y;
          acc.z = acc.z + term.z;
          acc.w = acc.w + 1.0f;
          out4[pix] = acc;
        }
      }
      const unsigned long long sm = __ballot(survive);
      if (survive) {
        const uint32_t slot = kPoolEntries - 1u - nReady - (uint32_t)__popcll(sm & laneBelow);
        s_pool[slot] = make_uint4(packPath(p, path, k + 1), __float_as_uint(L.x), __float_as_uint(L.y), __float_as_uint(L.z));
      }
      nReady += (uint32_t)__popcll(sm);
      __builtin_amdgcn_fence(__ATOMIC_RELEASE, "workgroup");
      __syncthreads();
    }
    const int empty = 64 - __popcll(travMask);
    if ((empty >= BDPT_WALK_REFILL || travMask == 0ull) && (nReady > 0 || !exhausted)) {
      const unsigned long long emptyMask = ~travMask;
      const uint32_t rank = (uint32_t)__popcll(emptyMask & laneBelow);
      const uint32_t fromReady = ((uint32_t)empty < nReady) ? (uint32_t)empty : nReady;
      bool got = false;
      uint32_t nid = 0;
      f3 dir = mk(0);
      if (!trav && rank < fromReady) {
        const uint4 r = s_pool[kPoolEntries - nReady + rank];
        nid = r.x;
        dir = mk(__uint_as_float(r.y), __uint_as_float(r.z), __uint_as_float(r.w));
        got = true;
      }
      __syncthreads();
      nReady -= fromReady;
      uint32_t want = (uint32_t)empty - fromReady;
      uint32_t taken = fromReady;
      while (want > 0 && !exhausted) {
        while (chunkPos >= chunkEnd && !exhausted) {
          const uint32_t* counts = (MASKED && vq < kNumSubQueues) ? M.walkEyeCount : P.qcount;
          const uint32_t nq = counts[(vq % kNumSubQueues) * kCursorStride];
          uint32_t base = nq;
          if (__hip_atomic_load(&head[vq * kCursorStride], __ATOMIC_RELAXED, __HIP_MEMORY_SCOPE_AGENT) < nq) {
            uint32_t share = (nq / wavesPerList + 15u) & ~15u;
            chunk = share < 16u ? 16u : (share > (uint32_t)BDPT_WALK_CHUNK ? (uint32_t)BDPT_WALK_CHUNK : share);
            if (lane == 0) base = atomicAdd(&head[vq * kCursorStride], chunk);
            base = (uint32_t)__builtin_amdgcn_readfirstlane((int)base);
          }
          if (base < nq) {
            chunkPos = base;
            chunkEnd = (base + chunk < nq) ? base + chunk : nq;
            tried = 0;
          } else {
            vq = (vq + 1 == 2u * kNumSubQueues) ? firstV : vq + 1;
            if (++tried >= numV) exhausted = true;
          }
        }
        if (exhausted) break;
        const uint32_t avail = chunkEnd - chunkPos;
        const uint32_t take = (want < avail) ? want : avail;
        if (!trav && !got && rank >= taken && rank < taken + take) {
          const uint32_t* items = (MASKED && vq < kNumSubQueues) ? M.walkEye : P.queue[0];
          const uint32_t p = items[(vq % kNumSubQueues) * P.pathSubCap + chunkPos + (rank - taken)];
          const int path = (int)(vq / kNumSubQueues);
          const float* rd = P.rayDir + (size_t)(path * 3) * P.Np + p;
          nid = packPath(p, path, (path == PATH_EYE) ? 1 : 0);
          dir = mk(rd[0], rd[P.Np], rd[2 * (size_t)P.Np]);
          got = true;
        }
        chunkPos += take;
        taken += take;
        want -= take;
      }
      if (got) {
        id = nid;
        travInit(T, ldPlane3(P, (int)((nid >> 24) & 1u), (int)(nid >> 25), F_POS, nid & 0xffffffu), dir, F.p.minT, 1.0e38f);
        trav = true;
      }
      travMask = __ballot(trav);
    }
    if (travMask == 0ull) {
      if (nParked == 0 && nReady == 0 && exhausted) break;
      continue;
    }
    bool finished = false;
#if BDPT_WALK_LEAF_WAIT > 0
    if (trav) {
#pragma unroll 1
      for (int kk = 0; kk < BDPT_WALK_NODE_BURST && T.cur >= 0; kk++) {
        if (COUNT) nNodes++;
        nodeStep<BDPT_WALK_ORDER, kWalkStackLds>(S, T, stk);
      }
    }
    {
      const unsigned long long waitMask = __ballot(trav && T.cur < 0), nodeMask = __ballot(trav && T.cur >= 0);
      const int waitNeed = (__popcll(waitMask | nodeMask) * BDPT_LEAF_WAIT_FRAC8 + 7) >> 3;
      if ((int)__popcll(waitMask) >= waitNeed || nodeMask == 0ull) {
        if (trav && T.cur < 0) {
          finished = (T.cur == kDone);
          if (!finished) {
            finished = leafStep<0, COUNT>(S, T, nTris, nAlpha);
            if (!finished) {
              T.cur = travPop<kWalkStackLds>(S, T, stk);
              finished = (T.cur == kDone);
            }
          }
        }
      }
    }
#else
    if (trav) {
      while (T.cur >= 0) {
        if (COUNT) nNodes++;
        nodeStep<BDPT_WALK_ORDER, kWalkStackLds>(S, T, stk);
      }
      finished = (T.cur == kDone);
      if (!finished) {
        finished = leafStep<0, COUNT>(S, T, nTris, nAlpha);
        if (!finished) {
          T.cur = travPop<kWalkStackLds>(S, T, stk);
          finished = (T.cur == kDone);
        }
      }
    }
#endif
    const unsigned long long finMask = __ballot(finished);
    if (finMask) {
      if (finished) {
        const bool miss = T.best.prim < 0;
        s_pool[nParked + (uint32_t)__popcll(finMask & laneBelow)] =
            (EXT && miss) ? make_uint4(id | kParkedMiss, __float_as_uint(T.d.x), __float_as_uint(T.d.y), __float_as_uint(T.d.z))
                          : make_uint4(id, (uint32_t)T.best.prim, __float_as_uint(T.best.u), __float_as_uint(T.best.v));
        trav = false;
      }
      nParked += (uint32_t)__popcll(finMask);
      __syncthreads();
    }
  }
  if (lane == 0) {
    if (nEye) atomicAdd(&F.counters->v[blockIdx.x % kCounterShards][C_RAYS_EYE], (unsigned long long)nEye);
    if (nLight) atomicAdd(&F.counters->v[blockIdx.x % kCounterShards][C_RAYS_LIGHT], (unsigned long long)nLight);
  }
  if (COUNT) {
    waveAddCount(F.counters, C_NODE_CLOSEST, nNodes);
    waveAddCount(F.counters, C_TRI_CLOSEST, nTris);
    waveAddCount(F.counters, C_ALPHA_CLOSEST, nAlpha);
  }
}

BD float evalGWithoutVPos(f3 posA, f3 nA, f3 posB, f3 nB) {
  const f3 vecAB = posB - posA;
  const float invLengthAB = 1.0f / length(vecAB);
  const f3 dirAB = vecAB * invLengthAB;
  const float cosA = fabsf(dot(nA, dirAB));
  const float cosB = fabsf(dot(nB, dirAB));
  return cosA * cosB * invLengthAB * invLengthAB;
}

__global__ __launch_bounds__(kWave) void mis_prefix_kernel(FrameDev F, PathBuf P) {
  BDPT_ONE_WAVE_PER_GROUP();
  bool act = false;
  uint32_t i = 0;
  if (!queueChunk(P.qcount, P.pathSubCap, act, i)) return;
  if (!act) return;
  const uint32_t p = P.queue[0][i];
  const int D = (int)F.p.maxDepth;
  const int eyeLast = P.eyeLast[p], lightLast = P.lightLast[p];
  f3 prevPos = ld3(F.cam.posW), prevN = normalize(ld3(F.cam.cameraW));
  float pE = 1.0f;
  P.misE[p] = pE;
  for (int x = 1; x <= D; x++) {
    f3 pos = mk(0), N = mk(0);
    float pdf = 0.0f;
    if (x <= eyeLast) {
      pos = ldPlane3(P, PATH_EYE, x, F_POS, p);
      N = ldPlane3(P, PATH_EYE, x, F_N, p);
      pdf = ldPlane1(P, PATH_EYE, x, F_PDF, p);
    }
    pE *= pdf * evalGWithoutVPos(prevPos, prevN, pos, N);
    P.misE[(size_t)x * P.Np + p] = pE;
    prevPos = pos;
    prevN = N;
  }
  prevPos = ldPlane3(P, PATH_LIGHT, 0, F_POS, p);
  prevN = ldPlane3(P, PATH_LIGHT, 0, F_N, p);
  float pL = ldPlane1(P, PATH_LIGHT, 0, F_PDF, p);
  P.misL[p] = pL;
  for (int x = 1; x <= D; x++) {
    f3 pos = mk(0), N = mk(0);
    float pdf = 0.0f;
    if (x <= lightLast) {
      pos = ldPlane3(P, PATH_LIGHT, x, F_POS, p);
      N = ldPlane3(P, PATH_LIGHT, x, F_N, p);
      pdf = ldPlane1(P, PATH_LIGHT, x, F_PDF, p);
    }
    pL *= pdf * evalGWithoutVPos(prevPos, prevN, pos, N);
    P.misL[(size_t)x * P.Np + p] = pL;
    prevPos = pos;
    prevN = N;
  }
}

BD float misWeight(const PathBuf& P, uint32_t p, int cameraIndex, int lightIndex, bool power) {
  const int totalLength = cameraIndex + lightIndex;
  float totalPdf = 0.0f, currentPdf = 1.0f;
  for (int i = 0; i <= totalLength; i++) {
    const int j = totalLength - i;
    const float pE = P.misE[(size_t)i * P.Np + p], pL = P.misL[(size_t)j * P.Np + p];
    const float term = power ? (pE * pE * pL * pL) : (pE * pL);
    totalPdf += term;
    if (j == lightIndex) currentPdf = term;
  }
  return currentPdf / totalPdf;
}
BD f3 applyStrategyWeight(const FrameDev& F, const PathBuf& P, uint32_t p, f3 v, int k, int cameraIndex, int lightIndex) {
  if (F.p.flags & (BDPT_PARAM_MIS_POWER | BDPT_PARAM_MIS_LINEAR))
    return v * misWeight(P, p, cameraIndex, lightIndex, (F.p.flags & BDPT_PARAM_MIS_POWER) != 0);
  return v / (float)k;
}

BD uint32_t emitRay(const PathBuf& P, int cls, bool active, f3 o, f3 d, float tmax, f3 contrib) {
  const unsigned long long mask = __ballot(active);
  uint32_t id = kNoRay;
  if (mask == 0ull) return id;
  const int lane = (int)(threadIdx.x & 63u);
  const int leader = __ffsll((long long)mask) - 1;
  uint32_t base = 0;
  const uint32_t q = blockIdx.x % kNumRaySubQueues;
  if (lane == leader) base = atomicAdd(&P.rayCount[(size_t)cls * kRayCursorBlock + q * kCursorStride], (uint32_t)__popcll(mask));
  base = (uint32_t)__shfl((int)base, leader);
  if (active) {
    id = P.rayBase[cls] + q * P.raySubCap[cls] + base + (uint32_t)__popcll(mask & ((1ull << lane) - 1ull));
    const size_t c = P.rayCap;
    float* r = P.rayQ + id;
    r[0] = o.x;
    r[c] = o.y;
    r[2 * c] = o.z;
    r[3 * c] = d.x;
    r[4 * c] = d.y;
    r[5 * c] = d.z;
    r[6 * c] = tmax;
    float* q = P.rayContrib + id;
    q[0] = contrib.x;
    q[c] = contrib.y;
    q[2 * c] = contrib.z;
  }
  return id;
}

template <bool GGX>
BD void loadConnVtx(const PathBuf& P, int path, int k, int last, uint32_t p, Vtx& v) {
  if (k > last) {
    v = zeroVtx();
    return;
  }
  loadSurf<GGX>(P, path, k, p, v);
}

template <int G>
BD bool queueGroup(const uint32_t* count, uint32_t subCap, bool& act, uint32_t& idx, int& g) {
  constexpr uint32_t kPix = kWave / G;
  const uint32_t q = blockIdx.x % kNumSubQueues, c0 = (blockIdx.x / kNumSubQueues) * kPix;
  const uint32_t n = count[q * kCursorStride];
  if (c0 >= n) return false;
  const uint32_t i = c0 + threadIdx.x / G;
  g = (int)(threadIdx.x % G);
  act = i < n;
  idx = q * subCap + i;
  return true;
}

template <bool GGX, int G, bool AREA>
BD void genNeeLane(const SceneDev& S, const FrameDev& F, const PathBuf& P, const AreaDev& A) {
  bool act = false;
  uint32_t i = 0;
  int t = 0;
  if (!queueGroup<G>(P.qcount, P.pathSubCap, act, i, t)) return;
  const int D = (int)F.p.maxDepth;
  const bool firstOfPixel = act && t == 0;
  act = act && t < D;
  const uint32_t p = act ? P.queue[0][i] : 0u;
  const int eyeLast = act ? (int)P.eyeLast[p] : 0;
  const float areaW = AREA ? areaTotal(A) : 0.0f;
  const int lightsCount = (int)S.numLights + ((AREA && areaW > 0.0f) ? 1 : 0);
  uint32_t seed = act ? P.seedL[p] : 0u;
  float r = 0.0f;
  for (int k = 0; k <= t; k++) r = nextRand(seed);
  bool emit = false, hinted = false;
  f3 pos = mk(0), L = mk(0), shade = mk(0);
  float distToLight = 0.0f;
  if (act && (t + 1) <= eyeLast) {
    int lightToSample = (int)(r * (float)lightsCount);
    if (lightToSample > lightsCount - 1) lightToSample = lightsCount - 1;
    Vtx v;
    loadSurf<GGX>(P, PATH_EYE, t + 1, p, v);
    pos = v.pos;
    f3 V = mk(0);
    if (GGX) V = ldPlane3(P, PATH_EYE, t + 1, F_V, p);
    const f3 prevColor = (t == 0) ? mk(1.0f) : ldPlane3(P, PATH_EYE, t, F_COL, p);
    f3 lightIntensity;
    const bool area = AREA && lightToSample == (int)S.numLights;
    if (area) {
      areaNee(S, A, areaW, seed, pos, L, distToLight, lightIntensity);
      distToLight = distToLight * (1.0f - 1e-4f);
    } else {
      getLightData(S.sc->lights[lightToSample], pos, L, lightIntensity, distToLight);
    }
    f3 direct = directIfVisible<GGX>((float)lightsCount, L, lightIntensity, v.N, V, v.dif, v.spec, v.rough);
    shade = clampVec(applyStrategyWeight(F, P, p, prevColor * direct, t + 2, t + 1, 0), F.p.clampUpper);
    emit = !allZero(shade);
    if (emit && !area && S.sc->lights[lightToSample].type != BDPT_LIGHT_DIRECTIONAL &&
        recOccludes(S, lightHint(S, lightToSample, ld3(S.sc->lights[lightToSample].posW), pos), pos, L, F.p.minT, distToLight)) {
      emit = false;
      hinted = true;
    }
  }
  const uint32_t id = emitRay(P, RAY_TERMS, emit, pos, L, distToLight, shade);
  if (act) P.slotRay[(size_t)t * P.Np + p] = id;
  waveAddCount(F.counters, C_RAYS_NEE, emit ? 1u : 0u);
  waveAddCount(F.counters, C_HINT_NEE, hinted ? 1u : 0u);
  waveAddCount(F.counters, C_PIX_VALID, firstOfPixel ? 1u : 0u);
}
template <bool GGX, int G>
__global__ __launch_bounds__(kWave) void gen_nee_kernel(SceneDev S, FrameDev F, PathBuf P) {
  BDPT_ONE_WAVE_PER_GROUP();
  genNeeLane<GGX, G, false>(S, F, P, AreaDev{});
}
template <bool GGX, int G>
__global__ __launch_bounds__(kWave) void gen_nee_area_kernel(SceneDev S, FrameDev F, PathBuf P, AreaDev A) {
  BDPT_ONE_WAVE_PER_GROUP();
  genNeeLane<GGX, G, true>(S, F, P, A);
}

template <bool GGX, int G>
__global__ __launch_bounds__(kWave) void gen_splat_kernel(SceneDev S, FrameDev F, PathBuf P) {
  BDPT_ONE_WAVE_PER_GROUP();
  bool act = false;
  uint32_t i = 0;
  int t = 0;
  if (!queueGroup<G>(P.qcount, P.pathSubCap, act, i, t)) return;
  const int D = (int)F.p.maxDepth;
  act = act && t < D;
  const uint32_t p = act ? P.queue[0][i] : 0u;
  const int real = act ? (int)P.lightReal[p] : 0;
  const SplatCam cam = splatCam(F.cam);
  bool emit = false, hinted = false;
  f3 pos = mk(0), dirToCamera = mk(0), shade = mk(0);
  float disToCamera = 0.0f;
  uint32_t target = kNoRay;
  if (act && t < real) {
    Vtx lv;
    loadSurf<GGX>(P, PATH_LIGHT, t + 1, p, lv);
    pos = lv.pos;
    dirToCamera = normalize(cam.pos - lv.pos);
    disToCamera = length(cam.pos - lv.pos);
    float fx = 0.0f, fy = 0.0f;
    emit = splatTarget(cam, dirToCamera, F.W, F.H, F.p.pixelJitter[0], F.p.pixelJitter[1], fx, fy);
    if (emit) {
      target = (uint32_t)splatIndex(F.sl, F.W, (uint32_t)(int)fx, (uint32_t)(int)fy);
      f3 vV = mk(0);
      if (GGX) vV = ldPlane3(P, PATH_LIGHT, t + 1, F_V, p);
      f3 fr;
      float Gt;
      splatTerm<GGX>(cam, lv, vV, dirToCamera, disToCamera, fr, Gt);
      f3 prevColor = ldPlane3(P, PATH_LIGHT, t, F_COL, p);
      shade = clampVec(applyStrategyWeight(F, P, p, (prevColor * fr) * Gt, t + 2, 0, t + 1), F.p.clampUpper);
      if (isnan3(shade)) shade = mk(0);
      if (F.hintPix && recOccludes(S, F.hintPix[(size_t)(uint32_t)(int)fy * F.W + (uint32_t)(int)fx], pos, dirToCamera, F.p.minT, disToCamera)) {
        emit = false;
        hinted = true;
      }
    }
  }
  const uint32_t id = emitRay(P, RAY_TERMS, emit, pos, dirToCamera, disToCamera, shade);
  if (act) {
    P.slotRay[(size_t)(D + t) * P.Np + p] = id;
    P.splatPix[(size_t)t * P.Np + p] = target;
  }
  waveAddCount(F.counters, C_RAYS_SPLAT, emit ? 1u : 0u);
  waveAddCount(F.counters, C_HINT_SPLAT, hinted ? 1u : 0u);
}

template <bool GGX, int G>
__global__ __launch_bounds__(kWave) void gen_connect_kernel(SceneDev S, FrameDev F, PathBuf P) {
  BDPT_ONE_WAVE_PER_GROUP();
  constexpr int kPix = kWave / G;
  __shared__ float4 s_light[kPix][G][4];
  __shared__ float4 s_eyePos[kPix][G];
  __shared__ uint8_t s_pair[G * (G - 1) / 2];
  bool act = false;
  uint32_t i = 0;
  int g = 0;
  if (!queueGroup<G>(P.qcount, P.pathSubCap, act, i, g)) return;
  const int e = (int)(threadIdx.x / G);
  const uint32_t p = act ? P.queue[0][i] : 0u;
  const int D = (int)F.p.maxDepth;
  const int eyeLast = act ? (int)P.eyeLast[p] : 0;
  const int lightLast = act ? (int)P.lightLast[p] : -1;
  const f3 camPos = ld3(F.cam.posW);
  const int cameraLength = g + 1;
  const bool camAct = act && cameraLength <= D - 1;
  const int nEval = (D * (D - 1)) / 2;
  for (int q = (int)threadIdx.x; q < nEval; q += kWave) {
    int c = 1, r = q;
    while (r >= D - c) {
      r -= D - c;
      c++;
    }
    s_pair[q] = (uint8_t)((c << 4) | (r + 1));
  }
  {
    float4 l0 = make_float4(0, 0, 0, 0), l1 = l0, l2 = l0, l3 = l0;
    if (act && g <= lightLast && g < D) {
      const float4* r = vtxPtr(P, PATH_LIGHT, g, p);
      l0 = r[0];
      l1 = r[1];
      l2 = r[2];
      if (GGX) l3 = r[3];
    }
    s_light[e][g][0] = l0;
    s_light[e][g][1] = l1;
    s_light[e][g][2] = l2;
    s_light[e][g][3] = l3;
  }
  Vtx ce = zeroVtx();
  f3 aE = mk(0), aL = mk(0);
  if (camAct) {
    loadConnVtx<GGX>(P, PATH_EYE, cameraLength, eyeLast, p, ce);
    if (cameraLength - 1 == 0)
      aE = mk(1.0f);
    else if (cameraLength - 1 <= eyeLast)
      aE = ldPlane3(P, PATH_EYE, cameraLength - 1, F_COL, p);
    aL = (cameraLength - 1 <= lightLast) ? ldPlane3(P, PATH_LIGHT, cameraLength - 1, F_COL, p) : mk(0);
  }
  s_eyePos[e][g] = make_float4(ce.pos.x, ce.pos.y, ce.pos.z, 0.0f);
  __syncthreads();
  f3 cprevPos = camPos;
  if (g > 0) {
    const float4 q = s_eyePos[e][g - 1];
    cprevPos = mk(q.x, q.y, q.z);
  }
  const f3 woE = normalize(cprevPos - ce.pos);
  if (camAct && cameraLength >= 2)
    P.slotRay[(size_t)(2 * D + ((cameraLength - 1) * cameraLength) / 2 - 1 + (cameraLength - 1)) * P.Np + p] = kNoRay;
  const int groupBase = (int)threadIdx.x - g;
  const int rounds = (nEval + G - 1) / G;
  uint32_t nConn = 0;
  for (int it = 0; it < rounds; it++) {
    const int ord = it * G + g;
    const bool pairAct = act && ord < nEval;
    const int cl = (ord < nEval) ? (int)s_pair[ord] : ((1 << 4) | 1);
    const int c = cl >> 4, lightLength = cl & 15, totalLength = c + lightLength;
    const int slot = 2 * D + ((totalLength - 1) * totalLength) / 2 - 1 + (c - 1);
    const int src = groupBase + c - 1;
    Vtx ev;
    ev.pos = mk(__shfl(ce.pos.x, src), __shfl(ce.pos.y, src), __shfl(ce.pos.z, src));
    ev.N = mk(__shfl(ce.N.x, src), __shfl(ce.N.y, src), __shfl(ce.N.z, src));
    ev.dif = mk(__shfl(ce.dif.x, src), __shfl(ce.dif.y, src), __shfl(ce.dif.z, src));
    if (GGX) {
      ev.spec = mk(__shfl(ce.spec.x, src), __shfl(ce.spec.y, src), __shfl(ce.spec.z, src));
      ev.rough = __shfl(ce.rough, src);
      ev.isSpec = __shfl(ce.isSpec ? 1 : 0, src) != 0;
    } else {
      ev.spec = mk(0);
      ev.rough = 0.0f;
      ev.isSpec = false;
    }
    const f3 aEs = mk(__shfl(aE.x, src), __shfl(aE.y, src), __shfl(aE.z, src));
    const f3 aLs = mk(__shfl(aL.x, src), __shfl(aL.y, src), __shfl(aL.z, src));
    const f3 woEs = mk(__shfl(woE.x, src), __shfl(woE.y, src), __shfl(woE.z, src));
    bool emit = false;
    f3 dirAB = mk(0), shade = mk(0);
    float lengthAB = 0.0f;
    if (pairAct) {
      const float4 q0 = s_light[e][lightLength][0], q1 = s_light[e][lightLength][1], q2 = s_light[e][lightLength][2];
      Vtx le;
      le.pos = mk(q0.x, q0.y, q0.z);
      le.N = mk(q1.x, q1.y, q1.z);
      le.dif = mk(q2.x, q2.y, q2.z);
      if (GGX) {
        const float4 q3 = s_light[e][lightLength][3];
        le.spec = mk(q3.x, q3.y, q3.z);
        le.rough = q0.w;
        le.isSpec = q1.w != 0.0f;
      } else {
        le.spec = mk(0);
        le.rough = 0.0f;
        le.isSpec = false;
      }
      const float4 qp = s_light[e][lightLength - 1][0];
      const f3 lprev = mk(qp.x, qp.y, qp.z);
      const f3 woL = normalize(lprev - le.pos);
      f3 cst;
      if (pairValue<GGX>(ev, woEs, le, woL, cst)) cst = (aLs * cst) * aEs;
      shade = clampVec(applyStrategyWeight(F, P, p, cst, totalLength, c, lightLength), F.p.clampUpper);
      if (isnan3(shade)) shade = mk(0);
      if (!allZero(shade)) {
        emit = true;
        pairRay(ev.pos, le.pos, dirAB, lengthAB);
      }
    }
    const uint32_t id = emitRay(P, RAY_PAIRS, emit, ev.pos, dirAB, lengthAB, shade);
    if (pairAct) P.slotRay[(size_t)slot * P.Np + p] = id;
    nConn += emit ? 1u : 0u;
  }
  waveAddCount(F.counters, C_RAYS_CONNECT, nConn);
}

constexpr int kGatherChunk = 8;
struct SlotChunk {
  uint32_t id[kGatherChunk];
  bool vis[kGatherChunk];
  float cx[kGatherChunk], cy[kGatherChunk], cz[kGatherChunk];
};
BD void loadSlotChunk(const PathBuf& P, uint32_t p, int slot0, int n, SlotChunk& c) {
  const size_t cap = P.rayCap;
#pragma unroll
  for (int j = 0; j < kGatherChunk; j++) c.id[j] = (j < n) ? P.slotRay[(size_t)(slot0 + j) * P.Np + p] : kNoRay;
#pragma unroll
  for (int j = 0; j < kGatherChunk; j++) c.vis[j] = (c.id[j] != kNoRay) && (P.rayVis[c.id[j]] != 0);
#pragma unroll
  for (int j = 0; j < kGatherChunk; j++) {
    c.cx[j] = c.cy[j] = c.cz[j] = 0.0f;
    if (c.vis[j]) {
      c.cx[j] = P.rayContrib[c.id[j]];
      c.cy[j] = P.rayContrib[cap + c.id[j]];
      c.cz[j] = P.rayContrib[2 * cap + c.id[j]];
    }
  }
}

template <bool GROUPS, bool MASKED>
BD bool gatherLane(const FrameDev& F, const PathBuf& P, const GroupDev& Gr, float* la, uint32_t p, uint32_t& nSplat, bool active) {
  bool pending = false;
  const bool sums = !MASKED || active;
  const size_t pix = P.pix[p];
  float4* out4 = reinterpret_cast<float4*>(F.out);
  float4 acc = out4[pix];
  const int D = (int)F.p.maxDepth;
  const int K = GROUPS ? (int)Gr.numGroups : 0;
  float ex = acc.x, ey = acc.y, ez = acc.z;
  int own = 0;
  int lightsCount = 0;
  if (GROUPS) {
    for (int r = 0; r < 3 * K; r++) la[r * kWave] = 0.0f;
    own = (int)Gr.groupOf[Gr.lightIdx[p]];
    const float areaW = Gr.areaW ? Gr.areaW[0] : 0.0f;
    lightsCount = (int)Gr.numLights + ((areaW > 0.0f) ? 1 : 0);
  }
  SlotChunk c;
  if (sums && !(F.p.flags & BDPT_PARAM_NO_NEE)) {
    uint32_t seed = GROUPS ? P.seedL[p] : 0u;
    for (int t0 = 0; t0 < D; t0 += kGatherChunk) {
      const int n = (D - t0 < kGatherChunk) ? D - t0 : kGatherChunk;
      loadSlotChunk(P, p, t0, n, c);
#pragma unroll
      for (int j = 0; j < kGatherChunk; j++)
        if (j < n) {
          acc.x = acc.x + c.cx[j];
          acc.y = acc.y + c.cy[j];
          acc.z = acc.z + c.cz[j];
          acc.w = acc.w + 1.0f;
          if (GROUPS) {
            int l = (int)(nextRand(seed) * (float)lightsCount);
            if (l > lightsCount - 1) l = lightsCount - 1;
            float* a = la + 3 * (int)Gr.groupOf[l] * kWave;
            a[0] = a[0] + c.cx[j];
            a[kWave] = a[kWave] + c.cy[j];
            a[2 * kWave] = a[2 * kWave] + c.cz[j];
            ex = ex + 0.0f;
            ey = ey + 0.0f;
            ez = ez + 0.0f;
          }
        }
    }
  }
  if (sums && !(F.p.flags & BDPT_PARAM_NO_CONNECT)) {
    const int nPairs = (int)numConnectPairs((uint32_t)D);
    bool sat = false;
    float ox = 0.0f, oy = 0.0f, oz = 0.0f;
    if (GROUPS) {
      ox = la[(3 * own) * kWave];
      oy = la[(3 * own + 1) * kWave];
      oz = la[(3 * own + 2) * kWave];
    }
    for (int s0 = 0; s0 < nPairs; s0 += kGatherChunk) {
      const int n = (nPairs - s0 < kGatherChunk) ? nPairs - s0 : kGatherChunk;
      loadSlotChunk(P, p, 2 * D + s0, n, c);
#pragma unroll
      for (int j = 0; j < kGatherChunk; j++)
        if (c.vis[j]) {
          acc.x = saturate(acc.x + c.cx[j]);
          acc.y = saturate(acc.y + c.cy[j]);
          acc.z = saturate(acc.z + c.cz[j]);
          acc.w = saturate(acc.w + 1.0f);
          if (GROUPS) {
            ox = saturate(ox + c.cx[j]);
            oy = saturate(oy + c.cy[j]);
            oz = saturate(oz + c.cz[j]);
          }
          sat = true;
        }
    }
    if (GROUPS) {
      if (sat) {
        for (int r = 0; r < 3 * K; r++) la[r * kWave] = saturate(la[r * kWave] + 0.0f);
        ex = saturate(ex + 0.0f);
        ey = saturate(ey + 0.0f);
        ez = saturate(ez + 0.0f);
      }
      la[(3 * own) * kWave] = ox;
      la[(3 * own + 1) * kWave] = oy;
      la[(3 * own + 2) * kWave] = oz;
    }
    pending = (!sat && nPairs > 0);
  }
  if (sums) out4[pix] = acc;
  if (GROUPS) {
    float4* g4 = reinterpret_cast<float4*>(Gr.planes) + pix;
    for (int k = 0; k < K; k++) g4[(size_t)k * Gr.framePix] = make_float4(la[(3 * k) * kWave], la[(3 * k + 1) * kWave], la[(3 * k + 2) * kWave], acc.w);
    g4[(size_t)K * Gr.framePix] = make_float4(ex, ey, ez, acc.w);
  }
  if (!(F.p.flags & BDPT_PARAM_NO_SPLAT)) {
    for (int t0 = 0; t0 < D; t0 += kGatherChunk) {
      const int n = (D - t0 < kGatherChunk) ? D - t0 : kGatherChunk;
      loadSlotChunk(P, p, D + t0, n, c);
      uint32_t target[kGatherChunk];
#pragma unroll
      for (int j = 0; j < kGatherChunk; j++) target[j] = c.vis[j] ? P.splatPix[(size_t)(t0 + j) * P.Np + p] : kNoRay;
#pragma unroll
      for (int j = 0; j < kGatherChunk; j++) {
        if (!c.vis[j] || target[j] == kNoRay) continue;
        unsigned long long* sp = F.splat + (size_t)target[j] * 4;
        unsigned long long* sv = GROUPS ? Gr.splat + ((size_t)own * Gr.framePix + target[j]) * 4 : sp;
        const unsigned long long qx = toFixed(c.cx[j]), qy = toFixed(c.cy[j]), qz = toFixed(c.cz[j]);
        if (qx) atomicAdd(&sv[0], qx);
        if (qy) atomicAdd(&sv[1], qy);
        if (qz) atomicAdd(&sv[2], qz);
        atomicAdd(&sp[3], 1ull);
        nSplat++;
      }
    }
  }
  return pending;
}

template <FrameKind V>
__global__ __launch_bounds__(kWave) void gather_kernel(FrameDev F, PathBuf P, uint32_t* __restrict__ lazyList,
                                                       uint32_t* __restrict__ lazyCount, FrameArg<V> A) {
  BDPT_ONE_WAVE_PER_GROUP();
  constexpr bool GROUPS = V == FrameKind::Groups, MASKED = V == FrameKind::Masked;
  extern __shared__ float s_acc[];
  bool act = false;
  uint32_t i = 0;
  if (!queueChunk(P.qcount, P.pathSubCap, act, i)) return;
  uint32_t nSplat = 0, p = 0;
  bool pending = false;
  if (act) {
    p = P.queue[0][i];
    pending = gatherLane<GROUPS, MASKED>(F, P, groupOf(A), GROUPS ? s_acc + threadIdx.x : nullptr, p, nSplat,
                                         !MASKED || maskOf(A).mask[P.pix[p]] != 0);
    if (pending) P.lazyCursor[p] = 0;
  }
  waveAddCount(F.counters, C_SPLATS, nSplat);
  wavePush(pending, p, lazyList, lazyCount, P.pathSubCap);
}

BD void pairFromOrdinal(int D, int ord, int& totalLength, int& cameraLength) {
  int t = 2;
  for (; t <= D; t++) {
    const int cnt = (t < D - 1) ? t : (D - 1);
    if (ord < cnt) break;
    ord -= cnt;
  }
  totalLength = t;
  cameraLength = ord + 1;
}

template <int G>
__global__ __launch_bounds__(kWave) void lazy_gen_kernel(FrameDev F, PathBuf P, const uint32_t* __restrict__ list,
                                                         const uint32_t* __restrict__ listCount, int batch) {
  BDPT_ONE_WAVE_PER_GROUP();
  bool act = false;
  uint32_t i = 0;
  int g = 0;
  if (!queueGroup<G>(listCount, P.pathSubCap, act, i, g)) return;
  const uint32_t p = act ? list[i] : 0u;
  const int D = (int)F.p.maxDepth;
  const int nPairs = (int)numConnectPairs((uint32_t)D);
  const int eyeLast = act ? (int)P.eyeLast[p] : 0, lightLast = act ? (int)P.lightLast[p] : -1;
  const bool lightGhost = act && (int)P.lightReal[p] < lightLast;
  const int lane = (int)(threadIdx.x & 63u), groupShift = lane - g;
  const unsigned long long groupMask = ((1ull << G) - 1ull) << groupShift, below = (1ull << lane) - 1ull;
  int base = act ? (int)P.lazyCursor[p] : nPairs;
  int cursor = base;
  int taken = 0;
  uint32_t nRays = 0;
  for (;;) {
    const bool live = act && taken < batch && base < nPairs;
    if (__ballot(live) == 0ull) break;
    const int ord = base + g;
    bool cand = false;
    int cameraLength = 0, lightLength = 0;
    if (live && ord < nPairs && P.slotRay[(size_t)(2 * D + ord) * P.Np + p] == kNoRay) {
      int totalLength = 0;
      pairFromOrdinal(D, ord, totalLength, cameraLength);
      lightLength = totalLength - cameraLength;
      const int cmin = (cameraLength <= eyeLast) ? cameraLength : eyeLast + 1;
      int lmin = (lightLength > lightLast) ? lightLast + 1 : ((lightGhost && lightLength == lightLast) ? lightLast - 1 : lightLength);
      if (cmin == 1 && lmin == 0) lmin = 1;
      cand = (cameraLength == cmin && lightLength == lmin);
    }
    const unsigned long long cm = __ballot(cand) & groupMask;
    const int rank = __popcll(cm & below), n = __popcll(cm);
    const bool emit = cand && taken + rank < batch;
    const unsigned long long lastM = __ballot(cand && taken + rank == batch - 1) & groupMask;
    f3 posA = mk(0), dirAB = mk(0);
    float lengthAB = 0.0f;
    if (emit) {
      posA = (cameraLength <= eyeLast) ? ldPlane3(P, PATH_EYE, cameraLength, F_POS, p) : mk(0);
      const f3 posB = (lightLength <= lightLast) ? ldPlane3(P, PATH_LIGHT, lightLength, F_POS, p) : mk(0);
      pairRay(posA, posB, dirAB, lengthAB);
    }
    const uint32_t id = emitRay(P, RAY_PAIRS, emit, posA, dirAB, lengthAB, mk(0));
    if (emit) P.lazyRay[(size_t)(taken + rank) * P.Np + p] = id;
    nRays += emit ? 1u : 0u;
    if (live) {
      if (lastM != 0ull) {
        cursor = base + (__ffsll((long long)lastM) - 1 - groupShift) + 1;
        taken = batch;
      } else {
        taken += n;
        base += G;
        cursor = base < nPairs ? base : nPairs;
      }
    }
  }
  if (act) {
    for (int b = taken + g; b < batch; b += G) P.lazyRay[(size_t)b * P.Np + p] = kNoRay;
    if (g == 0) P.lazyCursor[p] = (uint8_t)cursor;
  }
  waveAddCount(F.counters, C_RAYS_CONNECT, nRays);
  waveAddCount(F.counters, C_RAYS_LAZY, nRays);
}

template <bool GROUPS>
BD void lazyCheck(const FrameDev& F, const PathBuf& P, const GroupDev& Gr, const uint32_t* list, const uint32_t* listCount, int batch,
                  uint32_t* nextList, uint32_t* nextCount) {
  bool act = false;
  uint32_t i = 0;
  if (!queueChunk(listCount, P.pathSubCap, act, i)) return;
  bool again = false;
  uint32_t p = 0;
  if (act) {
    p = list[i];
    bool vis = false;
    for (int b = 0; b < batch; b++) {
      const uint32_t id = P.lazyRay[(size_t)b * P.Np + p];
      if (id != kNoRay && P.rayVis[id]) vis = true;
    }
    if (vis) {
      const size_t pix = P.pix[p];
      float4* out4 = reinterpret_cast<float4*>(F.out);
      float4 acc = out4[pix];
      acc.x = saturate(acc.x + 0.0f);
      acc.y = saturate(acc.y + 0.0f);
      acc.z = saturate(acc.z + 0.0f);
      acc.w = saturate(acc.w + 1.0f);
      out4[pix] = acc;
      if (GROUPS) {
        float4* g4 = reinterpret_cast<float4*>(Gr.planes) + pix;
        for (uint32_t k = 0; k <= Gr.numGroups; k++) {
          float4 o = g4[(size_t)k * Gr.framePix];
          o.x = saturate(o.x + 0.0f);
          o.y = saturate(o.y + 0.0f);
          o.z = saturate(o.z + 0.0f);
          o.w = saturate(o.w + 1.0f);
          g4[(size_t)k * Gr.framePix] = o;
        }
      }
    } else {
      const int nPairs = (int)numConnectPairs(F.p.maxDepth);
      again = (int)P.lazyCursor[p] < nPairs;
    }
  }
  wavePush(again, p, nextList, nextCount, P.pathSubCap);
}
template <FrameKind V>
__global__ __launch_bounds__(kWave) void lazy_check_kernel(FrameDev F, PathBuf P, const uint32_t* __restrict__ list,
                                                           const uint32_t* __restrict__ listCount, int batch,
                                                           uint32_t* __restrict__ nextList, uint32_t* __restrict__ nextCount, FrameArg<V> A) {
  BDPT_ONE_WAVE_PER_GROUP();
  lazyCheck<V == FrameKind::Groups>(F, P, groupOf(A), list, listCount, batch, nextList, nextCount);
}

__global__ void resolve_kernel(const unsigned long long* __restrict__ splat, bool tileLocal, uint32_t splatRow0, SplatLayout L,
                               float4* __restrict__ out, uint32_t W, const uint32_t* __restrict__ pixOf, uint32_t Np) {
  for (size_t p = (size_t)blockIdx.x * blockDim.x + threadIdx.x; p < Np; p += (size_t)gridDim.x * blockDim.x) {
    const size_t pix = pixOf[p];
    size_t sidx = p;
    if (!tileLocal) {
      const uint32_t y = (uint32_t)(pix / W), x = (uint32_t)(pix - (size_t)y * W);
      sidx = splatIndex(L, W, x, y) - (size_t)splatRow0 * W;
    }
    const ulonglong2 a = reinterpret_cast<const ulonglong2*>(splat + sidx * 4)[0];
    const ulonglong2 b = reinterpret_cast<const ulonglong2*>(splat + sidx * 4)[1];
    if (b.y == 0ull) continue;
    float4 o = out[pix];
    o.x = saturate(o.x + (float)a.x * 2.3283064365386963e-10f);
    o.y = saturate(o.y + (float)a.y * 2.3283064365386963e-10f);
    o.z = saturate(o.z + (float)b.x * 2.3283064365386963e-10f);
    o.w = saturate(o.w + (float)b.y);
    out[pix] = o;
  }
}

__global__ void resolve_masked_kernel(const unsigned long long* __restrict__ splat, float4* __restrict__ out, const uint8_t* __restrict__ mask,
                                      const uint32_t* __restrict__ pixOf, uint32_t Np) {
  for (size_t p = (size_t)blockIdx.x * blockDim.x + threadIdx.x; p < Np; p += (size_t)gridDim.x * blockDim.x) {
    const size_t pix = pixOf[p];
    if (mask[pix] == 0) continue;
    const ulonglong2 a = reinterpret_cast<const ulonglong2*>(splat + pix * 4)[0];
    const ulonglong2 b = reinterpret_cast<const ulonglong2*>(splat + pix * 4)[1];
    if (b.y == 0ull) continue;
    float4 o = out[pix];
    o.x = saturate(o.x + (float)a.x * 2.3283064365386963e-10f);
    o.y = saturate(o.y + (float)a.y * 2.3283064365386963e-10f);
    o.z = saturate(o.z + (float)b.x * 2.3283064365386963e-10f);
    o.w = saturate(o.w + (float)b.y);
    out[pix] = o;
  }
}

__global__ void resolve_groups_kernel(FrameDev F, const uint32_t* __restrict__ pixOf, uint32_t Np, GroupDev Gr) {
  constexpr float kInvFix = 2.3283064365386963e-10f;
  float4* out = reinterpret_cast<float4*>(F.out);
  for (size_t p = (size_t)blockIdx.x * blockDim.x + threadIdx.x; p < Np; p += (size_t)gridDim.x * blockDim.x) {
    const size_t pix = pixOf[p];
    const uint32_t y = (uint32_t)(pix / F.W), x = (uint32_t)(pix - (size_t)y * F.W);
    const size_t sidx = splatIndex(F.sl, F.W, x, y);
    const unsigned long long cnt = F.splat[sidx * 4 + 3];
    if (cnt == 0ull) continue;
    float4* g4 = reinterpret_cast<float4*>(Gr.planes) + pix;
    unsigned long long tx = 0, ty = 0, tz = 0;
    for (uint32_t k = 0; k <= Gr.numGroups; k++) {
      unsigned long long vx = 0, vy = 0, vz = 0;
      if (k < Gr.numGroups) {
        const unsigned long long* sv = Gr.splat + ((size_t)k * Gr.framePix + sidx) * 4;
        const ulonglong2 a = reinterpret_cast<const ulonglong2*>(sv)[0];
        vx = a.x;
        vy = a.y;
        vz = sv[2];
        tx += vx;
        ty += vy;
        tz += vz;
      }
      float4 o = g4[(size_t)k * Gr.framePix];
      o.x = saturate(o.x + (float)vx * kInvFix);
      o.y = saturate(o.y + (float)vy * kInvFix);
      o.z = saturate(o.z + (float)vz * kInvFix);
      o.w = saturate(o.w + (float)cnt);
      g4[(size_t)k * Gr.framePix] = o;
    }
    float4 o = out[pix];
    o.x = saturate(o.x + (float)tx * kInvFix);
    o.y = saturate(o.y + (float)ty * kInvFix);
    o.z = saturate(o.z + (float)tz * kInvFix);
    o.w = saturate(o.w + (float)cnt);
    out[pix] = o;
  }
}

__global__ void accumulate_kernel(float4* __restrict__ last, float4* __restrict__ cur, uint32_t accumCount, uint32_t maxAccum,
                                  uint64_t numTexels) {
  for (uint64_t i = (uint64_t)blockIdx.x * blockDim.x + threadIdx.x; i < numTexels; i += (uint64_t)gridDim.x * blockDim.x) {
    const float4 c = cur[i], pv = last[i];
    float4 r;
    if (accumCount < maxAccum) {
      const float a = (float)accumCount, b = (float)(accumCount + 1);
      r.x = (a * pv.x + c.x) / b;
      r.y = (a * pv.y + c.y) / b;
      r.z = (a * pv.z + c.z) / b;
      r.w = (a * pv.w + c.w) / b;
    } else {
      r = pv;
    }
    cur[i] = r;
    last[i] = r;
  }
}

__global__ void accumulate_tile_kernel(float4* __restrict__ last, float4* __restrict__ cur, uint32_t accumCount, uint32_t maxAccum,
                                       const uint32_t* __restrict__ pixOf, uint32_t Np) {
  for (size_t p = (size_t)blockIdx.x * blockDim.x + threadIdx.x; p < Np; p += (size_t)gridDim.x * blockDim.x) {
    const size_t i = pixOf[p];
    const float4 c = cur[i], pv = last[i];
    float4 r;
    if (accumCount < maxAccum) {
      const float a = (float)accumCount, b = (float)(accumCount + 1);
      r.x = (a * pv.x + c.x) / b;
      r.y = (a * pv.y + c.y) / b;
      r.z = (a * pv.z + c.z) / b;
      r.w = (a * pv.w + c.w) / b;
    } else {
      r = pv;
    }
    cur[i] = r;
    last[i] = r;
  }
}

__global__ void test_rng_kernel(const uint32_t* v0, const uint32_t* v1, uint32_t n, uint32_t draws, uint32_t* states, float* floats) {
  const uint32_t i = blockIdx.x * blockDim.x + threadIdx.x;
  if (i >= n) return;
  uint32_t s = initRand(v0[i], v1[i]);
  for (uint32_t k = 0; k < draws; k++) {
    float r = nextRand(s);
    states[(size_t)i * draws + k] = s;
    floats[(size_t)i * draws + k] = r;
  }
}
template <int MODE>
__global__ __launch_bounds__(kWave) void test_trace_kernel(SceneDev S, const float* rays, uint32_t n, int32_t* prim, float* tuv) {
  BDPT_ONE_WAVE_PER_GROUP();
  __shared__ int s_stack[kStackEntries * kWave];
  const uint32_t i = blockIdx.x * kWave + threadIdx.x;
  if (i >= n) return;
  const float* r = rays + (size_t)i * 8;
  uint32_t a = 0, b = 0;
  Hit h = traverse<MODE, false>(S, ld3(r), ld3(r + 3), r[6], r[7], s_stack + threadIdx.x, a, b);
  if (MODE != 2 && h.prim >= 0) {
    const bool named = h.rec < S.numRecs && (int)__float_as_uint(reinterpret_cast<const float4*>(S.recs)[(size_t)h.rec * kRecF4].w) == h.prim;
    if (!named) h.prim = -2;
  }
  prim[i] = h.prim;
  const bool rec = (MODE != 2) && h.prim >= 0;
  tuv[(size_t)i * 3] = rec ? h.t : 0.0f;
  tuv[(size_t)i * 3 + 1] = rec ? h.u : 0.0f;
  tuv[(size_t)i * 3 + 2] = rec ? h.v : 0.0f;
}
template <bool GGX>
__global__ void test_bsdf_kernel(const float* in, uint32_t n, bool fromLobe, float* out) {
  const uint32_t i = blockIdx.x * blockDim.x + threadIdx.x;
  if (i >= n) return;
  const float* p = in + (size_t)i * 20;
  f3 N = ld3(p), V = ld3(p + 3), Lq = ld3(p + 6), dif = ld3(p + 9), spec = ld3(p + 12);
  float rough = p[15];
  bool isSpec = p[16] != 0.0f;
  uint32_t seed = __float_as_uint(p[17]);
  f3 L;
  float pdf;
  bool sSpec;
  f3 w = sampleBRDF<GGX>(seed, N, N, V, dif, spec, rough, fromLobe, L, pdf, sSpec);
  f3 fr = evalBRDF<GGX>(V, Lq, N, N, dif, spec, rough, isSpec);
  float* o = out + (size_t)i * 16;
  o[0] = w.x;
  o[1] = w.y;
  o[2] = w.z;
  o[3] = L.x;
  o[4] = L.y;
  o[5] = L.z;
  o[6] = pdf;
  o[7] = sSpec ? 1.0f : 0.0f;
  o[8] = fr.x;
  o[9] = fr.y;
  o[10] = fr.z;
  o[11] = o[12] = o[13] = o[14] = o[15] = 0.0f;
}


static inline uint32_t blocksFor(uint64_t n) { return (uint32_t)((n + kWave - 1) / kWave); }
static inline uint32_t queueGrid(const PathBuf& P) { return (P.pathSubCap / kWave) * kNumSubQueues; }


template <class Fn>
static void withFlags(Fn&& fn) {
  fn();
}
template <class Fn, class... Flags>
static void withFlags(Fn&& fn, bool f, Flags... rest) {
  if (f)
    withFlags([&](auto... t) { fn(std::true_type{}, t...); }, rest...);
  else
    withFlags([&](auto... t) { fn(std::false_type{}, t...); }, rest...);
}
template <class Fn>
static void withKind(FrameKind kind, Fn&& fn) {
  if (kind == FrameKind::Groups)
    fn(std::integral_constant<FrameKind, FrameKind::Groups>{});
  else if (kind == FrameKind::Masked)
    fn(std::integral_constant<FrameKind, FrameKind::Masked>{});
  else
    fn(std::integral_constant<FrameKind, FrameKind::Plain>{});
}
template <FrameKind K>
static FrameArg<K> frameArg(const FrameVariant& V) {
  if constexpr (K == FrameKind::Groups)
    return V.groups;
  else if constexpr (K == FrameKind::Masked)
    return V.mask;
  else
    return NoArg{};
}

void launchGBuffer(const SceneDev& S, const GBufferDev& G, hipStream_t st) {
  const uint32_t Np = G.Np;
  if (!Np) return;
  withFlags([&](auto CNT) { launchWave(gbuffer_kernel<CNT>, blocksFor(Np), st, S, G); }, G.counters != nullptr);
}

__global__ void alpha_recs_kernel(SceneDev S, const uint32_t* __restrict__ alphaTris, uint32_t n, const unsigned long long* __restrict__ quadByTex,
                                  float4* __restrict__ out) {
  const uint32_t i = blockIdx.x * blockDim.x + threadIdx.x;
  if (i >= n) return;
  const uint32_t t = alphaTris[i];
  const float4* sr = S.shade + (size_t)t * kShadeRecF4;
  const float4 a1 = sr[1], b1 = sr[3], c1 = sr[5], m6 = sr[6];
  const uint32_t mid = __float_as_uint(m6.x);
  const bdpt_material& m = S.materials[mid];
  const uint32_t type = BDPT_FLAG_DIFFUSE_TYPE(m.flags);
  uint32_t mode = 0, tw = 0, th = 0, pow2 = 0;
  unsigned long long px = 0;
  if (type == BDPT_CHANNEL_UNUSED) {
    mode = 0;
  } else if (!alphaSamplesTexture(type, m.texBaseColor)) {
    mode = 1;
  } else {
    mode = 2;
    const TexDev td = S.matTex[(size_t)mid * 4];
    tw = td.w;
    th = td.h;
    pow2 = td.pow2;
    px = quadByTex[m.texBaseColor];
  }
  float4* r = out + (size_t)i * 4;
  r[0] = make_float4(a1.z, a1.w, b1.z, b1.w);
  r[1] = make_float4(c1.z, c1.w, m.alphaThreshold, m.baseColor[3]);
  r[2] = make_float4(__uint_as_float(mode), __uint_as_float(tw), __uint_as_float(th), __uint_as_float(pow2));
  r[3] = make_float4(__uint_as_float((uint32_t)(px & 0xffffffffull)), __uint_as_float((uint32_t)(px >> 32)), 0.0f, 0.0f);
}
void launchAlphaRecs(const SceneDev& S, const uint32_t* alphaTris, uint32_t n, const unsigned long long* quadByTex, float4* out, hipStream_t st) {
  if (!n) return;
  hipLaunchKernelGGL(alpha_recs_kernel, dim3((n + 255) / 256), dim3(256), 0, st, S, alphaTris, n, quadByTex, out);
}

void launchHintFill(const SceneDev& S, const GBufferDev& G, hipStream_t st) {
  if (!G.Np || !G.hintPix) return;
  launchWave(gbuffer_kernel<false, true>, (uint32_t)(blocksFor(G.Np)), st, S, G);
}

void launchLightMaps(const SceneDev& S, uint32_t* maps, uint32_t res, hipStream_t st) {
  const uint64_t n = (uint64_t)6 * res * res * S.numLights;
  if (!n) return;
  launchWave(light_map_kernel, (uint32_t)((n + kWave - 1) / kWave), st, S, maps, res);
}

void launchInitPaths(const SceneDev& S, const FrameDev& F, const PathBuf& P, const FrameVariant& V, hipStream_t st) {
  if (!P.Np) return;
  if (V.area.n) {
    withKind(V.kind, [&](auto K) {
      withFlags([&](auto GGX) { launchWave(init_paths_area_kernel<GGX, K>, blocksFor(P.Np), st, S, F, P, frameArg<K>(V), V.area); },
                F.p.matIndex == 0);
    });
    return;
  }
  withKind(V.kind, [&](auto K) {
    withFlags([&](auto GGX) { launchWave(init_paths_kernel<GGX, K>, blocksFor(P.Np), st, S, F, P, frameArg<K>(V)); }, F.p.matIndex == 0);
  });
}

void launchWalk(const SceneDev& S, const FrameDev& F, const PathBuf& P, const FrameVariant& V, LaunchGrids& G, int numCUs,
                hipStream_t st) {
  if (!P.Np || F.p.maxDepth < 1) return;
  const bool cnt = (F.p.flags & BDPT_PARAM_COUNTERS) != 0, ggx = F.p.matIndex == 0;
  const bool ext = (F.p.flags & (BDPT_PARAM_ENV_ON_MISS | BDPT_PARAM_EMISSIVE_HITS)) != 0, masked = V.kind == FrameKind::Masked;
  uint32_t& g = G.walk[(masked ? 8 : 0) + (ext ? 4 : 0) + (ggx ? 2 : 0) + (cnt ? 1 : 0)];
  const uint32_t need = blocksFor((uint64_t)2 * P.Np);
  withFlags(
      [&](auto GGX, auto CNT, auto EXT, auto MASKED) {
        const auto kernel = walk_kernel<GGX, CNT, EXT, MASKED>;
        if (!g) g = persistentGrid(kernel, numCUs);
        launchWave(kernel, std::min(g, need), st, S, F, P, P.qhead, frameArg<MASKED ? FrameKind::Masked : FrameKind::Plain>(V));
      },
      ggx, cnt, ext, masked);
}

void launchMisPrefix(const FrameDev& F, const PathBuf& P, hipStream_t st) {
  if (!P.Np) return;
  launchWave(mis_prefix_kernel, (uint32_t)(queueGrid(P)), st, F, P);
}
void launchGenNee(const SceneDev& S, const FrameDev& F, const PathBuf& P, const AreaDev& A, hipStream_t st) {
  if (!P.Np) return;
  if (A.n) {
    withFlags([&](auto GGX, auto WIDE) { launchWave(gen_nee_area_kernel<GGX, WIDE ? 16 : 8>, queueGrid(P) * (WIDE ? 16 : 8), st, S, F, P, A); },
              F.p.matIndex == 0, P.D1 > 9);
    return;
  }
  withFlags([&](auto GGX, auto WIDE) { launchWave(gen_nee_kernel<GGX, WIDE ? 16 : 8>, queueGrid(P) * (WIDE ? 16 : 8), st, S, F, P); },
            F.p.matIndex == 0, P.D1 > 9);
}
void launchGenSplat(const SceneDev& S, const FrameDev& F, const PathBuf& P, hipStream_t st) {
  if (!P.Np || (F.p.flags & BDPT_PARAM_NO_SPLAT)) return;
  withFlags([&](auto GGX, auto WIDE) { launchWave(gen_splat_kernel<GGX, WIDE ? 16 : 8>, queueGrid(P) * (WIDE ? 16 : 8), st, S, F, P); },
            F.p.matIndex == 0, P.D1 > 9);
}
void launchGenConnect(const SceneDev& S, const FrameDev& F, const PathBuf& P, hipStream_t st) {
  if (!P.Np || (F.p.flags & BDPT_PARAM_NO_CONNECT) || F.p.maxDepth < 2) return;
  withFlags([&](auto GGX, auto WIDE) { launchWave(gen_connect_kernel<GGX, WIDE ? 16 : 8>, queueGrid(P) * (WIDE ? 16 : 8), st, S, F, P); },
            F.p.matIndex == 0, P.D1 > 9);
}

void launchTraceShadow(const SceneDev& S, const FrameDev& F, const PathBuf& P, int cls, LaunchGrids& G, int numCUs, hipStream_t st) {
  if (!P.Np) return;
  const bool cnt = (F.p.flags & BDPT_PARAM_COUNTERS) != 0;
  RayQueue Q{P.rayQ + P.rayBase[cls], P.rayCap, P.raySubCap[cls], kNumRaySubQueues, P.rayCount + (size_t)cls * kRayCursorBlock,
             P.rayHead + (size_t)cls * kRayCursorBlock};
  uint8_t* vis = P.rayVis + P.rayBase[cls];
  uint32_t& g = G.shadow[cnt ? 1 : 0];
  withFlags(
      [&](auto CNT) {
        if (!g) g = persistentGrid(trace_shadow_kernel<CNT>, numCUs);
        launchWave(trace_shadow_kernel<CNT>, g, st, S, Q, vis, F.counters, F.p.minT);
      },
      cnt);
}

void launchGather(const FrameDev& F, const PathBuf& P, const FrameVariant& V, uint32_t* lazyList, uint32_t* lazyCount, hipStream_t st) {
  if (!P.Np) return;
  const size_t lds = V.kind == FrameKind::Groups ? (size_t)3 * std::max(V.groups.numGroups, 1u) * kWave * sizeof(float) : 0;
  withKind(V.kind, [&](auto K) { launchWaveLds(gather_kernel<K>, queueGrid(P), lds, st, F, P, lazyList, lazyCount, frameArg<K>(V)); });
}
void launchLazyGen(const FrameDev& F, const PathBuf& P, const uint32_t* list, const uint32_t* listCount, int batch, hipStream_t st) {
  if (!P.Np) return;
  withFlags([&](auto WIDE) { launchWave(lazy_gen_kernel<WIDE ? 16 : 8>, queueGrid(P) * (WIDE ? 16 : 8), st, F, P, list, listCount, batch); },
            P.D1 > 9);
}
void launchLazyCheck(const FrameDev& F, const PathBuf& P, const FrameVariant& V, const uint32_t* list, const uint32_t* listCount,
                     int batch, uint32_t* nextList, uint32_t* nextCount, hipStream_t st) {
  if (!P.Np) return;
  if (V.kind == FrameKind::Groups)
    launchWave(lazy_check_kernel<FrameKind::Groups>, queueGrid(P), st, F, P, list, listCount, batch, nextList, nextCount, V.groups);
  else
    launchWave(lazy_check_kernel<FrameKind::Plain>, queueGrid(P), st, F, P, list, listCount, batch, nextList, nextCount, NoArg{});
}

void launchResolve(const unsigned long long* splat, bool tileLocal, uint32_t splatRow0, const SplatLayout& L, float* out, uint32_t W,
                   const uint32_t* pix, uint32_t Np, hipStream_t st) {
  if (!Np) return;
  const uint32_t grid = (uint32_t)std::min<uint64_t>(((uint64_t)Np + 255) / 256, 2048);
  hipLaunchKernelGGL(resolve_kernel, dim3(grid), dim3(256), 0, st, splat, tileLocal, splatRow0, L, reinterpret_cast<float4*>(out), W, pix,
                     Np);
}
void launchFrameResolve(const FrameDev& F, const PathBuf& P, const FrameVariant& V, hipStream_t st) {
  if (!P.Np) return;
  const uint32_t grid = (uint32_t)std::min<uint64_t>(((uint64_t)P.Np + 255) / 256, 2048);
  if (V.kind == FrameKind::Groups)
    hipLaunchKernelGGL(resolve_groups_kernel, dim3(grid), dim3(256), 0, st, F, P.pix, P.Np, V.groups);
  else if (V.kind == FrameKind::Masked)
    hipLaunchKernelGGL(resolve_masked_kernel, dim3(grid), dim3(256), 0, st, F.splat, reinterpret_cast<float4*>(F.out), V.mask.mask, P.pix, P.Np);
  else
    launchResolve(F.splat, false, 0, F.sl, F.out, F.W, P.pix, P.Np, st);
}
void launchAccumulate(float* last, float* cur, uint32_t accumCount, uint32_t maxAccum, uint64_t numTexels, hipStream_t st) {
  if (!numTexels) return;
  const uint32_t grid = (uint32_t)std::min<uint64_t>((numTexels + 255) / 256, 2048);
  hipLaunchKernelGGL(accumulate_kernel, dim3(grid), dim3(256), 0, st, reinterpret_cast<float4*>(last),
                     reinterpret_cast<float4*>(cur), accumCount, maxAccum, numTexels);
}
void launchAccumulateTile(float* last, float* cur, uint32_t accumCount, uint32_t maxAccum, const uint32_t* pix, uint32_t Np,
                          hipStream_t st) {
  if (!Np) return;
  const uint32_t grid = (uint32_t)std::min<uint64_t>(((uint64_t)Np + 255) / 256, 2048);
  hipLaunchKernelGGL(accumulate_tile_kernel, dim3(grid), dim3(256), 0, st, reinterpret_cast<float4*>(last), reinterpret_cast<float4*>(cur),
                     accumCount, maxAccum, pix, Np);
}
template <class T>
__global__ void tile_pack_kernel(const T* __restrict__ frame, T* __restrict__ packed, const uint32_t* __restrict__ pix, uint32_t Np) {
  const uint32_t i = blockIdx.x * blockDim.x + threadIdx.x;
  if (i < Np) packed[i] = frame[pix[i]];
}
template <class T>
__global__ void tile_unpack_kernel(const T* __restrict__ packed, T* __restrict__ frame, uint32_t W, uint32_t H, uint32_t R, uint32_t owners,
                                   uint32_t owner, uint32_t packedRows) {
  const size_t i = (size_t)blockIdx.x * blockDim.x + threadIdx.x;
  if (i >= (size_t)packedRows * W) return;
  const uint32_t r = (uint32_t)(i / W), x = (uint32_t)(i - (size_t)r * W);
  const uint32_t y = ((r / R) * owners + owner) * R + r % R;
  if (y < H) frame[(size_t)y * W + x] = packed[i];
}
void launchTilePack(const void* frame, void* packed, uint32_t bpp, const uint32_t* pix, uint32_t Np, hipStream_t st) {
  if (!Np) return;
  const dim3 g((Np + 255) / 256), b(256);
  if (bpp == 16)
    hipLaunchKernelGGL(tile_pack_kernel<uint4>, g, b, 0, st, (const uint4*)frame, (uint4*)packed, pix, Np);
  else if (bpp == 8)
    hipLaunchKernelGGL(tile_pack_kernel<uint2>, g, b, 0, st, (const uint2*)frame, (uint2*)packed, pix, Np);
  else
    hipLaunchKernelGGL(tile_pack_kernel<uint32_t>, g, b, 0, st, (const uint32_t*)frame, (uint32_t*)packed, pix, Np);
}
void launchTileUnpack(const void* packed, void* frame, uint32_t bpp, uint32_t W, uint32_t H, uint32_t R, uint32_t owners, uint32_t owner,
                      uint32_t packedRows, hipStream_t st) {
  const size_t n = (size_t)packedRows * W;
  if (!n) return;
  const dim3 g((uint32_t)((n + 255) / 256)), b(256);
  if (bpp == 16)
    hipLaunchKernelGGL(tile_unpack_kernel<uint4>, g, b, 0, st, (const uint4*)packed, (uint4*)frame, W, H, R, owners, owner, packedRows);
  else if (bpp == 8)
    hipLaunchKernelGGL(tile_unpack_kernel<uint2>, g, b, 0, st, (const uint2*)packed, (uint2*)frame, W, H, R, owners, owner, packedRows);
  else
    hipLaunchKernelGGL(tile_unpack_kernel<uint32_t>, g, b, 0, st, (const uint32_t*)packed, (uint32_t*)frame, W, H, R, owners, owner, packedRows);
}

void launchTestRng(const uint32_t* v0, const uint32_t* v1, uint32_t n, uint32_t draws, uint32_t* states, float* floats,
                   hipStream_t st) {
  if (!n) return;
  hipLaunchKernelGGL(test_rng_kernel, dim3((n + 255) / 256), dim3(256), 0, st, v0, v1, n, draws, states, floats);
}
void launchTestTrace(const SceneDev& S, const float* rays, uint32_t n, int mode, int32_t* prim, float* tuv, hipStream_t st) {
  if (!n) return;
  if (mode == 0)
    launchWave(test_trace_kernel<0>, (uint32_t)(blocksFor(n)), st, S, rays, n, prim, tuv);
  else if (mode == 1)
    launchWave(test_trace_kernel<1>, (uint32_t)(blocksFor(n)), st, S, rays, n, prim, tuv);
  else
    launchWave(test_trace_kernel<2>, (uint32_t)(blocksFor(n)), st, S, rays, n, prim, tuv);
}
void launchTestTraceShadow(const SceneDev& S, const float* planes, uint32_t cap, const uint32_t* count, uint32_t* head, uint8_t* vis,
                           DevCounters* counters, float tmin, int numCUs, hipStream_t st) {
  RayQueue Q{planes, cap, cap, 1u, count, head};
  const uint32_t g = persistentGrid(trace_shadow_kernel<true>, numCUs);
  launchWave(trace_shadow_kernel<true>, (uint32_t)(g), st, S, Q, vis, counters, tmin);
}
void launchTestBsdf(const float* in, uint32_t n, uint32_t matIndex, float* out, hipStream_t st) {
  if (!n) return;
  const bool fromLobe = (matIndex & 2u) != 0;
  if ((matIndex & 1u) == 0)
    hipLaunchKernelGGL(test_bsdf_kernel<true>, dim3((n + 255) / 256), dim3(256), 0, st, in, n, fromLobe, out);
  else
    hipLaunchKernelGGL(test_bsdf_kernel<false>, dim3((n + 255) / 256), dim3(256), 0, st, in, n, fromLobe, out);
}

}
```

Before: 4776.

## Track emitted shadow-ray slots with per-pixel bitmasks and per-round cursor blocks

Generation kernels now record per-pixel bitmasks of which NEE, splat and connection slots actually emitted a ray. Gather, lazy_gen and lazy_check use these masks or counts instead of reading and clearing kNoRay sentinels in slotRay and lazyRay. Each lazy round gets its own ray-cursor block, so the two per-round memsets go away, and lazy rays skip writing their zero contribution. This trades extra mask buffers and ballot/shuffle work for fewer scattered global reads and writes and fewer small launches.

```diff
diff --git a/fyp-bidirectionalpathtracer_amd/csrc/api.cpp b/fyp-bidirectionalpathtracer_amd/csrc/api.cpp
--- a/fyp-bidirectionalpathtracer_amd/csrc/api.cpp
+++ b/fyp-bidirectionalpathtracer_amd/csrc/api.cpp
@@ -30,7 +30,7 @@
 constexpr size_t kLazyBlocks = kMaxLazyRounds + 2;
 constexpr size_t kEyeCountBlock = kLazyBlocks - 1;
 static_assert(kEyeCountBlock > (size_t)kMaxLazyRounds, "the eye list's cursor block must be one no lazy round uses");
-constexpr size_t kCursorWords = (kCountBlocks + kHeadBlocks + kLazyBlocks) * kCursorBlock + 4 * kRayCursorBlock;
+constexpr size_t kCursorWords = (kCountBlocks + kHeadBlocks + kLazyBlocks) * kCursorBlock + 2 * (size_t)kRayCursorBlocks * kRayCursorBlock;
 }
 
 struct bdpt_ctx {
@@ -1532,7 +1532,7 @@
   P.qhead = P.qcount + kCountBlocks * kCursorBlock;
   P.lazyCount = P.qhead + kHeadBlocks * kCursorBlock;
   P.rayCount = P.lazyCount + kLazyBlocks * kCursorBlock;
-  P.rayHead = P.rayCount + 2 * kRayCursorBlock;
+  P.rayHead = P.rayCount + (size_t)kRayCursorBlocks * kRayCursorBlock;
   {
     const uint32_t D = std::max<uint32_t>(maxDepth, 1);
     const uint64_t slots = (uint64_t)2 * D + numConnectPairs(D);
@@ -1561,6 +1561,9 @@
     if ((rc = devAlloc(c, c->frameAllocs, &P.rayContrib, (size_t)3 * cap))) return rc;
     if ((rc = devAlloc(c, c->frameAllocs, &P.rayVis, (size_t)cap))) return rc;
     if ((rc = devAlloc(c, c->frameAllocs, &P.slotRay, (size_t)slots * np))) return rc;
+    if ((rc = devAlloc(c, c->frameAllocs, &P.neeMask, np))) return rc;
+    if ((rc = devAlloc(c, c->frameAllocs, &P.splatMask, np))) return rc;
+    if ((rc = devAlloc(c, c->frameAllocs, &P.pairMask, (size_t)std::max<uint32_t>(pairMaskWords(D), 1) * np))) return rc;
     if ((rc = devAlloc(c, c->frameAllocs, &P.splatPix, (size_t)D * np))) return rc;
     c->lazyRounds = np >= (1u << 18) ? 3 : 2;
     if (const char* e = std::getenv("BDPT_LAZY_ROUNDS")) {
@@ -1572,6 +1575,7 @@
     if ((rc = devAlloc(c, c->frameAllocs, &P.misL, (size_t)(D + 1) * np))) return rc;
     if ((rc = devAlloc(c, c->frameAllocs, &P.lazyCursor, np))) return rc;
     if ((rc = devAlloc(c, c->frameAllocs, &P.lazyRay, (size_t)std::max<uint32_t>(batch, 1) * np))) return rc;
+    if ((rc = devAlloc(c, c->frameAllocs, &P.lazyN, np))) return rc;
   }
   c->hintPix = nullptr;
   c->hintCamValid = false;
@@ -1698,14 +1702,11 @@
       left -= batch;
       uint32_t* list = P.queue[1 + (r & 1)];
       uint32_t* next = P.queue[1 + ((r + 1) & 1)];
-      HIPCHK(c, hipMemsetAsync(P.rayCount + (size_t)RAY_PAIRS * kRayCursorBlock, 0, kRayCursorBlock * sizeof(uint32_t), st));
-      HIPCHK(c, hipMemsetAsync(P.rayHead + (size_t)RAY_PAIRS * kRayCursorBlock, 0, kRayCursorBlock * sizeof(uint32_t), st));
-      launchLazyGen(F, P, list, P.lazyCount + (size_t)r * kCursorBlock, batch, st);
+      launchLazyGen(F, P, list, P.lazyCount + (size_t)r * kCursorBlock, batch, r + 1, st);
       stageMark(c, st, "lazy_gen");
-      launchTraceShadow(c->S, F, P, RAY_PAIRS, c->grids, c->numCUs, st);
+      launchTraceShadow(c->S, F, P, RAY_PAIRS, r + 1, c->grids, c->numCUs, st);
       stageMark(c, st, "lazy_trace");
-      launchLazyCheck(F, P, V, list, P.lazyCount + (size_t)r * kCursorBlock, batch, next, P.lazyCount + (size_t)(r + 1) * kCursorBlock,
-                      st);
+      launchLazyCheck(F, P, V, list, P.lazyCount + (size_t)r * kCursorBlock, next, P.lazyCount + (size_t)(r + 1) * kCursorBlock, st);
     }
     stageMark(c, st, "lazy_check");
   }
@@ -1783,7 +1784,7 @@
     stageMark(c, st, "gen_splat");
     launchGenConnect(c->S, F, PE, st);
     stageMark(c, st, "gen_connect");
-    launchTraceShadow(c->S, F, P, RAY_TERMS, c->grids, c->numCUs, st);
+    launchTraceShadow(c->S, F, P, RAY_TERMS, 0, c->grids, c->numCUs, st);
     stageMark(c, st, "trace_terms");
   } else {
     HIPCHK(c, hipEventRecord(c->evFork, st));
@@ -1800,12 +1801,12 @@
     stageMark(c, st, "gen_nee");
     HIPCHK(c, hipStreamWaitEvent(st, c->evSplat, 0));
     stageMark(c, st, "splat_wait");
-    launchTraceShadow(c->S, F, P, RAY_TERMS, c->grids, c->numCUs, st);
+    launchTraceShadow(c->S, F, P, RAY_TERMS, 0, c->grids, c->numCUs, st);
     stageMark(c, st, "trace_terms");
     HIPCHK(c, hipStreamWaitEvent(st, c->evJoin, 0));
     stageMark(c, st, "connect_wait");
   }
-  launchTraceShadow(c->S, F, P, RAY_PAIRS, c->grids, c->numCUs, st);
+  launchTraceShadow(c->S, F, P, RAY_PAIRS, 0, c->grids, c->numCUs, st);
   stageMark(c, st, "trace_pairs");
   launchGather(F, P, V, P.queue[1], P.lazyCount, st);
   stageMark(c, st, "gather");
diff --git a/fyp-bidirectionalpathtracer_amd/csrc/kernels.h b/fyp-bidirectionalpathtracer_amd/csrc/kernels.h
--- a/fyp-bidirectionalpathtracer_amd/csrc/kernels.h
+++ b/fyp-bidirectionalpathtracer_amd/csrc/kernels.h
@@ -85,6 +85,13 @@
   return n;
 }
 
+constexpr int kMaxPairMaskWords = 5;
+inline __host__ __device__ uint32_t pairMaskWords(uint32_t D) { return (numConnectPairs(D) + 31u) / 32u; }
+constexpr int kLazyBatchDiv = 8;
+constexpr int kMaxLazyRounds = 8;
+constexpr uint32_t kRayCursorBlocks = 2 + kMaxLazyRounds;
+inline __host__ __device__ uint32_t rayCursorBlock(int cls, int pairBlock) { return cls == RAY_TERMS ? 0u : 1u + (uint32_t)pairBlock; }
+
 struct PathBuf {
   float* v;
   float* rayDir;
@@ -106,11 +113,15 @@
   uint32_t raySubCap[2];
   uint32_t rayBase[2];
   uint32_t* slotRay;
+  uint16_t* neeMask;
+  uint16_t* splatMask;
+  uint32_t* pairMask;
   uint32_t* splatPix;
   float* misE;
   float* misL;
   uint8_t* lazyCursor;
   uint32_t* lazyRay;
+  uint8_t* lazyN;
   uint32_t* lazyCount;
   uint32_t rayCap;
   uint32_t Np, D1;
@@ -217,7 +228,8 @@
 void launchGenNee(const SceneDev& S, const FrameDev& F, const PathBuf& P, const AreaDev& A, hipStream_t st);
 void launchGenSplat(const SceneDev& S, const FrameDev& F, const PathBuf& P, hipStream_t st);
 void launchGenConnect(const SceneDev& S, const FrameDev& F, const PathBuf& P, hipStream_t st);
-void launchTraceShadow(const SceneDev& S, const FrameDev& F, const PathBuf& P, int rayClass, LaunchGrids& G, int numCUs, hipStream_t st);
+void launchTraceShadow(const SceneDev& S, const FrameDev& F, const PathBuf& P, int rayClass, int pairBlock, LaunchGrids& G, int numCUs,
+                       hipStream_t st);
 void launchTraceRays(const SceneDev& S, const float4* rays, uint32_t cap, const uint32_t* count, unsigned long long* cursor, int mode,
                      float4* hits, uint8_t* vis, LaunchGrids& G, int numCUs, hipStream_t st);
 void launchCameraRays(const bdpt_camera& cam, const bdpt_gbuffer_params& gp, uint32_t W, uint32_t H, float4* rays, hipStream_t st);
@@ -268,11 +280,10 @@
 };
 void launchSplatAdd(const SplatAddDev& A, hipStream_t st);
 void launchGather(const FrameDev& F, const PathBuf& P, const FrameVariant& V, uint32_t* lazyList, uint32_t* lazyCount, hipStream_t st);
-void launchLazyGen(const FrameDev& F, const PathBuf& P, const uint32_t* list, const uint32_t* listCount, int batch, hipStream_t st);
+void launchLazyGen(const FrameDev& F, const PathBuf& P, const uint32_t* list, const uint32_t* listCount, int batch, int pairBlock,
+                   hipStream_t st);
 void launchLazyCheck(const FrameDev& F, const PathBuf& P, const FrameVariant& V, const uint32_t* list, const uint32_t* listCount,
-                     int batch, uint32_t* nextList, uint32_t* nextCount, hipStream_t st);
-constexpr int kLazyBatchDiv = 8;
-constexpr int kMaxLazyRounds = 8;
+                     uint32_t* nextList, uint32_t* nextCount, hipStream_t st);
 void launchResolve(const unsigned long long* splat, bool tileLocal, uint32_t splatRow0, const SplatLayout& L, float* out, uint32_t W,
                    const uint32_t* pix, uint32_t Np, hipStream_t st);
 void launchFrameResolve(const FrameDev& F, const PathBuf& P, const FrameVariant& V, hipStream_t st);
diff --git a/fyp-bidirectionalpathtracer_amd/csrc/kernels.hip b/fyp-bidirectionalpathtracer_amd/csrc/kernels.hip
--- a/fyp-bidirectionalpathtracer_amd/csrc/kernels.hip
+++ b/fyp-bidirectionalpathtracer_amd/csrc/kernels.hip
@@ -226,8 +226,8 @@
       P.eyeLast[p] = 0;
       if (GROUPS) {
         float4* g4 = reinterpret_cast<float4*>(Gr.planes) + pix;
-        for (uint32_t k = 0; k < Gr.numGroups; k++) g4[(size_t)k * Gr.framePix] = make_float4(0.0f, 0.0f, 0.0f, 1.0f);
-        g4[(size_t)Gr.numGroups * Gr.framePix] = make_float4(dr, dg, db, 1.0f);
+        for (uint32_t k = 0; k <= Gr.numGroups; k++, g4 += Gr.framePix)
+          *g4 = (k == Gr.numGroups) ? make_float4(dr, dg, db, 1.0f) : make_float4(0.0f, 0.0f, 0.0f, 1.0f);
       }
     } else {
       float nx, ny, nz, nw, sr, sg, sb, sa, er, eg, eb, ea;
@@ -657,7 +657,10 @@
   return v / (float)k;
 }
 
-BD uint32_t emitRay(const PathBuf& P, int cls, bool active, f3 o, f3 d, float tmax, f3 contrib) {
+template <bool CONTRIB = true>
+BD uint32_t emitRay(const PathBuf& P, uint32_t cb, bool active, f3 o, f3 d, float tmax, f3 contrib) {
+  static_assert(RAY_TERMS == 0 && RAY_PAIRS == 1, "rayCursorBlock: block 0 is RAY_TERMS', every other block RAY_PAIRS'");
+  const int cls = cb == 0u ? RAY_TERMS : RAY_PAIRS;
   const unsigned long long mask = __ballot(active);
   uint32_t id = kNoRay;
   if (mask == 0ull) return id;
@@ -665,7 +668,7 @@
   const int leader = __ffsll((long long)mask) - 1;
   uint32_t base = 0;
   const uint32_t q = blockIdx.x % kNumRaySubQueues;
-  if (lane == leader) base = atomicAdd(&P.rayCount[(size_t)cls * kRayCursorBlock + q * kCursorStride], (uint32_t)__popcll(mask));
+  if (lane == leader) base = atomicAdd(&P.rayCount[(size_t)cb * kRayCursorBlock + q * kCursorStride], (uint32_t)__popcll(mask));
   base = (uint32_t)__shfl((int)base, leader);
   if (active) {
     id = P.rayBase[cls] + q * P.raySubCap[cls] + base + (uint32_t)__popcll(mask & ((1ull << lane) - 1ull));
@@ -678,10 +681,12 @@
     r[4 * c] = d.y;
     r[5 * c] = d.z;
     r[6 * c] = tmax;
-    float* q = P.rayContrib + id;
-    q[0] = contrib.x;
-    q[c] = contrib.y;
-    q[2 * c] = contrib.z;
+    if (CONTRIB) {
+      float* q = P.rayContrib + id;
+      q[0] = contrib.x;
+      q[c] = contrib.y;
+      q[2 * c] = contrib.z;
+    }
   }
   return id;
 }
@@ -706,6 +711,12 @@
   act = i < n;
   idx = q * subCap + i;
   return true;
+}
+
+template <int G>
+BD uint32_t groupBallot(bool v, int g) {
+  const int groupShift = (int)(threadIdx.x & 63u) - g;
+  return (uint32_t)((__ballot(v) >> groupShift) & ((1ull << G) - 1ull));
 }
 
 template <bool GGX, int G, bool AREA>
@@ -753,8 +764,10 @@
       hinted = true;
     }
   }
-  const uint32_t id = emitRay(P, RAY_TERMS, emit, pos, L, distToLight, shade);
-  if (act) P.slotRay[(size_t)t * P.Np + p] = id;
+  const uint32_t id = emitRay(P, rayCursorBlock(RAY_TERMS, 0), emit, pos, L, distToLight, shade);
+  if (emit) P.slotRay[(size_t)t * P.Np + p] = id;
+  const uint32_t termMask = groupBallot<G>(emit, t);
+  if (firstOfPixel) P.neeMask[p] = (uint16_t)termMask;
   waveAddCount(F.counters, C_RAYS_NEE, emit ? 1u : 0u);
   waveAddCount(F.counters, C_HINT_NEE, hinted ? 1u : 0u);
   waveAddCount(F.counters, C_PIX_VALID, firstOfPixel ? 1u : 0u);
@@ -810,11 +823,13 @@
       }
     }
   }
-  const uint32_t id = emitRay(P, RAY_TERMS, emit, pos, dirToCamera, disToCamera, shade);
-  if (act) {
+  const uint32_t id = emitRay(P, rayCursorBlock(RAY_TERMS, 0), emit, pos, dirToCamera, disToCamera, shade);
+  if (emit) {
     P.slotRay[(size_t)(D + t) * P.Np + p] = id;
     P.splatPix[(size_t)t * P.Np + p] = target;
   }
+  const uint32_t termMask = groupBallot<G>(emit, t);
+  if (act && t == 0) P.splatMask[p] = (uint16_t)termMask;
   waveAddCount(F.counters, C_RAYS_SPLAT, emit ? 1u : 0u);
   waveAddCount(F.counters, C_HINT_SPLAT, hinted ? 1u : 0u);
 }
@@ -823,6 +838,8 @@
 __global__ __launch_bounds__(kWave) void gen_connect_kernel(SceneDev S, FrameDev F, PathBuf P) {
   BDPT_ONE_WAVE_PER_GROUP();
   constexpr int kPix = kWave / G;
+  constexpr int kW = G == 8 ? 2 : kMaxPairMaskWords;
+  static_assert((G * (G - 1)) / 2 + (G - 1) - 1 < 32 * kW, "the highest slot ordinal at depth G has a bit in the lane's words");
   __shared__ float4 s_light[kPix][G][4];
   __shared__ float4 s_eyePos[kPix][G];
   __shared__ uint8_t s_pair[G * (G - 1) / 2];
@@ -879,8 +896,9 @@
     cprevPos = mk(q.x, q.y, q.z);
   }
   const f3 woE = normalize(cprevPos - ce.pos);
-  if (camAct && cameraLength >= 2)
-    P.slotRay[(size_t)(2 * D + ((cameraLength - 1) * cameraLength) / 2 - 1 + (cameraLength - 1)) * P.Np + p] = kNoRay;
+  uint32_t bits[kW];
+#pragma unroll
+  for (int w = 0; w < kW; w++) bits[w] = 0u;
   const int groupBase = (int)threadIdx.x - g;
   const int rounds = (nEval + G - 1) / G;
   uint32_t nConn = 0;
@@ -938,9 +956,24 @@
         pairRay(ev.pos, le.pos, dirAB, lengthAB);
       }
     }
-    const uint32_t id = emitRay(P, RAY_PAIRS, emit, ev.pos, dirAB, lengthAB, shade);
-    if (pairAct) P.slotRay[(size_t)slot * P.Np + p] = id;
+    const uint32_t id = emitRay(P, rayCursorBlock(RAY_PAIRS, 0), emit, ev.pos, dirAB, lengthAB, shade);
+    if (emit) {
+      P.slotRay[(size_t)slot * P.Np + p] = id;
+      const int refOrd = slot - 2 * D;
+#pragma unroll
+      for (int w = 0; w < kW; w++)
+        if ((refOrd >> 5) == w) bits[w] |= 1u << (refOrd & 31);
+    }
     nConn += emit ? 1u : 0u;
+  }
+  {
+    const int nWords = (int)pairMaskWords((uint32_t)D);
+#pragma unroll
+    for (int w = 0; w < kW; w++) {
+#pragma unroll
+      for (int d = 1; d < G; d <<= 1) bits[w] |= (uint32_t)__shfl_xor((int)bits[w], d);
+      if (act && g == 0 && w < nWords) P.pairMask[(size_t)w * P.Np + p] = bits[w];
+    }
   }
   waveAddCount(F.counters, C_RAYS_CONNECT, nConn);
 }
@@ -951,10 +984,8 @@
   bool vis[kGatherChunk];
   float cx[kGatherChunk], cy[kGatherChunk], cz[kGatherChunk];
 };
-BD void loadSlotChunk(const PathBuf& P, uint32_t p, int slot0, int n, SlotChunk& c) {
+BD void loadChunkRays(const PathBuf& P, SlotChunk& c) {
   const size_t cap = P.rayCap;
-#pragma unroll
-  for (int j = 0; j < kGatherChunk; j++) c.id[j] = (j < n) ? P.slotRay[(size_t)(slot0 + j) * P.Np + p] : kNoRay;
 #pragma unroll
   for (int j = 0; j < kGatherChunk; j++) c.vis[j] = (c.id[j] != kNoRay) && (P.rayVis[c.id[j]] != 0);
 #pragma unroll
@@ -966,6 +997,23 @@
       c.cz[j] = P.rayContrib[2 * cap + c.id[j]];
     }
   }
+}
+BD void loadSlotChunk(const PathBuf& P, uint32_t p, int slot0, uint32_t have, SlotChunk& c) {
+#pragma unroll
+  for (int j = 0; j < kGatherChunk; j++) c.id[j] = ((have >> j) & 1u) ? P.slotRay[(size_t)(slot0 + j) * P.Np + p] : kNoRay;
+  loadChunkRays(P, c);
+}
+BD void loadMaskChunk(const PathBuf& P, uint32_t p, int slot0, unsigned long long& m, SlotChunk& c) {
+#pragma unroll
+  for (int j = 0; j < kGatherChunk; j++) {
+    c.id[j] = kNoRay;
+    if (m != 0ull) {
+      const int b = __ffsll((long long)m) - 1;
+      m &= m - 1ull;
+      c.id[j] = P.slotRay[(size_t)(slot0 + b) * P.Np + p];
+    }
+  }
+  loadChunkRays(P, c);
 }
 
 template <bool GROUPS, bool MASKED>
@@ -989,9 +1037,10 @@
   SlotChunk c;
   if (sums && !(F.p.flags & BDPT_PARAM_NO_NEE)) {
     uint32_t seed = GROUPS ? P.seedL[p] : 0u;
+    const uint32_t neeMask = P.neeMask[p];
     for (int t0 = 0; t0 < D; t0 += kGatherChunk) {
       const int n = (D - t0 < kGatherChunk) ? D - t0 : kGatherChunk;
-      loadSlotChunk(P, p, t0, n, c);
+      loadSlotChunk(P, p, t0, neeMask >> t0, c);
 #pragma unroll
       for (int j = 0; j < kGatherChunk; j++)
         if (j < n) {
@@ -1022,23 +1071,28 @@
       oy = la[(3 * own + 1) * kWave];
       oz = la[(3 * own + 2) * kWave];
     }
-    for (int s0 = 0; s0 < nPairs; s0 += kGatherChunk) {
-      const int n = (nPairs - s0 < kGatherChunk) ? nPairs - s0 : kGatherChunk;
-      loadSlotChunk(P, p, 2 * D + s0, n, c);
+    const int nWords = (int)pairMaskWords((uint32_t)D);
+    for (int k = 0; 2 * k < nWords; k++) {
+      const uint32_t lo = P.pairMask[(size_t)(2 * k) * P.Np + p];
+      const uint32_t hi = (2 * k + 1 < nWords) ? P.pairMask[(size_t)(2 * k + 1) * P.Np + p] : 0u;
+      unsigned long long m = ((unsigned long long)hi << 32) | lo;
+      while (m != 0ull) {
+        loadMaskChunk(P, p, 2 * D + 64 * k, m, c);
 #pragma unroll
-      for (int j = 0; j < kGatherChunk; j++)
-        if (c.vis[j]) {
-          acc.x = saturate(acc.x + c.cx[j]);
-          acc.y = saturate(acc.y + c.cy[j]);
-          acc.z = saturate(acc.z + c.cz[j]);
-          acc.w = saturate(acc.w + 1.0f);
-          if (GROUPS) {
-            ox = saturate(ox + c.cx[j]);
-            oy = saturate(oy + c.cy[j]);
-            oz = saturate(oz + c.cz[j]);
+        for (int j = 0; j < kGatherChunk; j++)
+          if (c.vis[j]) {
+            acc.x = saturate(acc.x + c.cx[j]);
+            acc.y = saturate(acc.y + c.cy[j]);
+            acc.z = saturate(acc.z + c.cz[j]);
+            acc.w = saturate(acc.w + 1.0f);
+            if (GROUPS) {
+              ox = saturate(ox + c.cx[j]);
+              oy = saturate(oy + c.cy[j]);
+              oz = saturate(oz + c.cz[j]);
+            }
+            sat = true;
           }
-          sat = true;
-        }
+      }
     }
     if (GROUPS) {
       if (sat) {
@@ -1060,9 +1114,9 @@
     g4[(size_t)K * Gr.framePix] = make_float4(ex, ey, ez, acc.w);
   }
   if (!(F.p.flags & BDPT_PARAM_NO_SPLAT)) {
+    const uint32_t splatMask = P.splatMask[p];
     for (int t0 = 0; t0 < D; t0 += kGatherChunk) {
-      const int n = (D - t0 < kGatherChunk) ? D - t0 : kGatherChunk;
-      loadSlotChunk(P, p, D + t0, n, c);
+      loadSlotChunk(P, p, D + t0, splatMask >> t0, c);
       uint32_t target[kGatherChunk];
 #pragma unroll
       for (int j = 0; j < kGatherChunk; j++) target[j] = c.vis[j] ? P.splatPix[(size_t)(t0 + j) * P.Np + p] : kNoRay;
@@ -1117,7 +1171,7 @@
 
 template <int G>
 __global__ __launch_bounds__(kWave) void lazy_gen_kernel(FrameDev F, PathBuf P, const uint32_t* __restrict__ list,
-                                                         const uint32_t* __restrict__ listCount, int batch) {
+                                                         const uint32_t* __restrict__ listCount, int batch, uint32_t cursorBlock) {
   BDPT_ONE_WAVE_PER_GROUP();
   bool act = false;
   uint32_t i = 0;
@@ -1130,6 +1184,8 @@
   const bool lightGhost = act && (int)P.lightReal[p] < lightLast;
   const int lane = (int)(threadIdx.x & 63u), groupShift = lane - g;
   const unsigned long long groupMask = ((1ull << G) - 1ull) << groupShift, below = (1ull << lane) - 1ull;
+  static_assert(kMaxPairMaskWords <= 8, "a group's lanes hold the pixel's mask words");
+  const uint32_t maskWord = (act && g < (int)pairMaskWords((uint32_t)D)) ? P.pairMask[(size_t)g * P.Np + p] : 0u;
   int base = act ? (int)P.lazyCursor[p] : nPairs;
   int cursor = base;
   int taken = 0;
@@ -1140,7 +1196,8 @@
     const int ord = base + g;
     bool cand = false;
     int cameraLength = 0, lightLength = 0;
-    if (live && ord < nPairs && P.slotRay[(size_t)(2 * D + ord) * P.Np + p] == kNoRay) {
+    const uint32_t word = (uint32_t)__shfl((int)maskWord, groupShift + ((ord >> 5) & (G - 1)));
+    if (live && ord < nPairs && !((word >> (ord & 31)) & 1u)) {
       int totalLength = 0;
       pairFromOrdinal(D, ord, totalLength, cameraLength);
       lightLength = totalLength - cameraLength;
@@ -1160,7 +1217,7 @@
       const f3 posB = (lightLength <= lightLast) ? ldPlane3(P, PATH_LIGHT, lightLength, F_POS, p) : mk(0);
       pairRay(posA, posB, dirAB, lengthAB);
     }
-    const uint32_t id = emitRay(P, RAY_PAIRS, emit, posA, dirAB, lengthAB, mk(0));
+    const uint32_t id = emitRay<false>(P, cursorBlock, emit, posA, dirAB, lengthAB, mk(0));
     if (emit) P.lazyRay[(size_t)(taken + rank) * P.Np + p] = id;
     nRays += emit ? 1u : 0u;
     if (live) {
@@ -1175,15 +1232,17 @@
     }
   }
   if (act) {
-    for (int b = taken + g; b < batch; b += G) P.lazyRay[(size_t)b * P.Np + p] = kNoRay;
-    if (g == 0) P.lazyCursor[p] = (uint8_t)cursor;
+    if (g == 0) {
+      P.lazyCursor[p] = (uint8_t)cursor;
+      P.lazyN[p] = (uint8_t)taken;
+    }
   }
   waveAddCount(F.counters, C_RAYS_CONNECT, nRays);
   waveAddCount(F.counters, C_RAYS_LAZY, nRays);
 }
 
 template <bool GROUPS>
-BD void lazyCheck(const FrameDev& F, const PathBuf& P, const GroupDev& Gr, const uint32_t* list, const uint32_t* listCount, int batch,
+BD void lazyCheck(const FrameDev& F, const PathBuf& P, const GroupDev& Gr, const uint32_t* list, const uint32_t* listCount,
                   uint32_t* nextList, uint32_t* nextCount) {
   bool act = false;
   uint32_t i = 0;
@@ -1193,9 +1252,10 @@
   if (act) {
     p = list[i];
     bool vis = false;
-    for (int b = 0; b < batch; b++) {
+    const int n = (int)P.lazyN[p];
+    for (int b = 0; b < n; b++) {
       const uint32_t id = P.lazyRay[(size_t)b * P.Np + p];
-      if (id != kNoRay && P.rayVis[id]) vis = true;
+      if (P.rayVis[id]) vis = true;
     }
     if (vis) {
       const size_t pix = P.pix[p];
@@ -1226,10 +1286,10 @@
 }
 template <FrameKind V>
 __global__ __launch_bounds__(kWave) void lazy_check_kernel(FrameDev F, PathBuf P, const uint32_t* __restrict__ list,
-                                                           const uint32_t* __restrict__ listCount, int batch,
+                                                           const uint32_t* __restrict__ listCount,
                                                            uint32_t* __restrict__ nextList, uint32_t* __restrict__ nextCount, FrameArg<V> A) {
   BDPT_ONE_WAVE_PER_GROUP();
-  lazyCheck<V == FrameKind::Groups>(F, P, groupOf(A), list, listCount, batch, nextList, nextCount);
+  lazyCheck<V == FrameKind::Groups>(F, P, groupOf(A), list, listCount, nextList, nextCount);
 }
 
 __global__ void resolve_kernel(const unsigned long long* __restrict__ splat, bool tileLocal, uint32_t splatRow0, SplatLayout L,
@@ -1548,11 +1608,13 @@
             F.p.matIndex == 0, P.D1 > 9);
 }
 
-void launchTraceShadow(const SceneDev& S, const FrameDev& F, const PathBuf& P, int cls, LaunchGrids& G, int numCUs, hipStream_t st) {
+void launchTraceShadow(const SceneDev& S, const FrameDev& F, const PathBuf& P, int cls, int pairBlock, LaunchGrids& G, int numCUs,
+                       hipStream_t st) {
   if (!P.Np) return;
   const bool cnt = (F.p.flags & BDPT_PARAM_COUNTERS) != 0;
-  RayQueue Q{P.rayQ + P.rayBase[cls], P.rayCap, P.raySubCap[cls], kNumRaySubQueues, P.rayCount + (size_t)cls * kRayCursorBlock,
-             P.rayHead + (size_t)cls * kRayCursorBlock};
+  const size_t cb = rayCursorBlock(cls, pairBlock);
+  RayQueue Q{P.rayQ + P.rayBase[cls], P.rayCap, P.raySubCap[cls], kNumRaySubQueues, P.rayCount + cb * kRayCursorBlock,
+             P.rayHead + cb * kRayCursorBlock};
   uint8_t* vis = P.rayVis + P.rayBase[cls];
   uint32_t& g = G.shadow[cnt ? 1 : 0];
   withFlags(
@@ -1568,18 +1630,20 @@
   const size_t lds = V.kind == FrameKind::Groups ? (size_t)3 * std::max(V.groups.numGroups, 1u) * kWave * sizeof(float) : 0;
   withKind(V.kind, [&](auto K) { launchWaveLds(gather_kernel<K>, queueGrid(P), lds, st, F, P, lazyList, lazyCount, frameArg<K>(V)); });
 }
-void launchLazyGen(const FrameDev& F, const PathBuf& P, const uint32_t* list, const uint32_t* listCount, int batch, hipStream_t st) {
+void launchLazyGen(const FrameDev& F, const PathBuf& P, const uint32_t* list, const uint32_t* listCount, int batch, int pairBlock,
+                   hipStream_t st) {
   if (!P.Np) return;
-  withFlags([&](auto WIDE) { launchWave(lazy_gen_kernel<WIDE ? 16 : 8>, queueGrid(P) * (WIDE ? 16 : 8), st, F, P, list, listCount, batch); },
+  withFlags([&](auto WIDE) { launchWave(lazy_gen_kernel<WIDE ? 16 : 8>, queueGrid(P) * (WIDE ? 16 : 8), st, F, P, list, listCount, batch,
+                                          rayCursorBlock(RAY_PAIRS, pairBlock)); },
             P.D1 > 9);
 }
 void launchLazyCheck(const FrameDev& F, const PathBuf& P, const FrameVariant& V, const uint32_t* list, const uint32_t* listCount,
-                     int batch, uint32_t* nextList, uint32_t* nextCount, hipStream_t st) {
+                     uint32_t* nextList, uint32_t* nextCount, hipStream_t st) {
   if (!P.Np) return;
   if (V.kind == FrameKind::Groups)
-    launchWave(lazy_check_kernel<FrameKind::Groups>, queueGrid(P), st, F, P, list, listCount, batch, nextList, nextCount, V.groups);
+    launchWave(lazy_check_kernel<FrameKind::Groups>, queueGrid(P), st, F, P, list, listCount, nextList, nextCount, V.groups);
   else
-    launchWave(lazy_check_kernel<FrameKind::Plain>, queueGrid(P), st, F, P, list, listCount, batch, nextList, nextCount, NoArg{});
+    launchWave(lazy_check_kernel<FrameKind::Plain>, queueGrid(P), st, F, P, list, listCount, nextList, nextCount, NoArg{});
 }
 
 void launchResolve(const unsigned long long* splat, bool tileLocal, uint32_t splatRow0, const SplatLayout& L, float* out, uint32_t W,
```

After: 4833, median of 6. 1.2% higher.
